# zli96/DF-GNN

Hardware: AMD Instinct MI355X
Metric: edges/s (fwd+bwd) fused GT conv, PATTERN bs=1024 dim=128 (higher is better)
Workload: dtype f32; 1 GPU; GT conv 'hyper' fwd+bwd, PATTERN-like batch bs=1024 dim=128 heads=1 (BASELINE.json configs[2]); training_pair=attn_edge in rank order (dfgnn_gt_hyper_fwd_ranked / dfgnn_gt_bwd_ranked), nodes_per_gpu=120490, edges_per_gpu=6288908, total_edges=6288908, parallelism=graph-sharded x1 (weak scaling), no data-path collective

## Files before the change

df-gnn_amd/csrc/dfgnn_dense.hpp:

```cpp
#pragma once
#include "dfgnn_block.hpp"

namespace dfgnn {

typedef _Float16 h16;
typedef __attribute__((ext_vector_type(8))) _Float16 hx8;
typedef __attribute__((ext_vector_type(4))) _Float16 hx4;
typedef __fp16 fp16x4_raw __attribute__((__vector_size__(4 * sizeof(__fp16))));
typedef __attribute__((address_space(3))) fp16x4_raw *lds_hx4_ptr;

#if defined(DFGNN_LDS_CHECK)
__attribute__((used)) static __device__ unsigned g_lds_report[4];
__device__ __forceinline__ void lds_check(const void *p, unsigned bytes, int line) {
#if defined(__HIP_DEVICE_COMPILE__)
  if (!__builtin_amdgcn_is_shared(p)) return;
  const unsigned end = (unsigned)(size_t)p + bytes;
  const unsigned lim = __builtin_amdgcn_groupstaticsize() + ((const unsigned *)__builtin_amdgcn_implicitarg_ptr())[30];
  if (end > lim && atomicAdd(&g_lds_report[0], 1u) == 0u) {
    g_lds_report[1] = (unsigned)line;
    g_lds_report[2] = end;
    g_lds_report[3] = lim;
  }
#endif
}
#define DFGNN_LDS_AT(p, bytes) ::dfgnn::lds_check((p), (bytes), __LINE__)
void lds_report_register(const void *symbol);
namespace {
struct LdsReportReg {
  LdsReportReg() { lds_report_register(HIP_SYMBOL(g_lds_report)); }
} g_lds_report_reg;
}
#else
#define DFGNN_LDS_AT(p, bytes) ((void)0)
#endif

struct Pow2Scale {
  float s, inv;
};
__device__ __forceinline__ Pow2Scale pow2_scale(float amax) {
  const int b = min(max((__builtin_amdgcn_readfirstlane(__float_as_int(amax)) >> 23) & 0xFF, 15), 254);
  return Pow2Scale{__int_as_float((268 - b) << 23), __int_as_float((b - 14) << 23)};
}
constexpr float kUnitScale = 16384.f, kUnitScaleInv = 1.f / 16384.f;

__device__ __forceinline__ void split_hx8(const float4 &a, const float4 &b, float s, hx8 &hi, hx8 &lo) {
  const float x[8] = {a.x, a.y, a.z, a.w, b.x, b.y, b.z, b.w};
#pragma unroll
  for (int j = 0; j < 8; ++j) {
    const h16 h = (h16)(x[j] * s);
    hi[j] = h;
    lo[j] = (h16)fmaf(x[j], s, -(float)h);
  }
}
__device__ __forceinline__ float absmax8(const float4 &a, const float4 &b) {
  return fmaxf(fmaxf(fmaxf(fabsf(a.x), fabsf(a.y)), fmaxf(fabsf(a.z), fabsf(a.w))),
               fmaxf(fmaxf(fabsf(b.x), fabsf(b.y)), fmaxf(fabsf(b.z), fabsf(b.w))));
}

constexpr int kDenseThreads = 512;
constexpr int kDenseWaves = kDenseThreads / kWave;
constexpr int kDenseChunkRows = 128;
constexpr int kDenseWideRows = 160;
constexpr int kDensePre = 16;

template <int F>
struct DenseCfg {
  static constexpr int RS = F + 16;
  static constexpr int KT = F / 32;
  static constexpr int FT = F / 16;
};

template <class T>
__device__ __forceinline__ const T &ld32(const T *base, unsigned idx) {
  DFGNN_LDS_AT(reinterpret_cast<const char *>(base) + (size_t)(idx * (unsigned)sizeof(T)), (unsigned)sizeof(T));
  return *reinterpret_cast<const T *>(reinterpret_cast<const char *>(base) + (size_t)(idx * (unsigned)sizeof(T)));
}
__device__ __forceinline__ float4 ld32_f4(const float *base, unsigned idx) {
  DFGNN_LDS_AT(reinterpret_cast<const char *>(base) + (size_t)(idx * 4u), 16u);
  return *reinterpret_cast<const float4 *>(reinterpret_cast<const char *>(base) + (size_t)(idx * 4u));
}
__device__ __forceinline__ void st32_f4(float *base, unsigned idx, const float4 &v) {
  DFGNN_LDS_AT(reinterpret_cast<char *>(base) + (size_t)(idx * 4u), 16u);
  *reinterpret_cast<float4 *>(reinterpret_cast<char *>(base) + (size_t)(idx * 4u)) = v;
}
#ifndef DFGNN_NT_LOADS
#define DFGNN_NT_LOADS 1
#endif
template <class T>
__device__ __forceinline__ T ld32_once(const T *base, unsigned idx) {
  const T *p = reinterpret_cast<const T *>(reinterpret_cast<const char *>(base) + (size_t)(idx * (unsigned)sizeof(T)));
#if DFGNN_NT_LOADS
  return __builtin_nontemporal_load(p);
#else
  return *p;
#endif
}
__device__ __forceinline__ float4 ld32_f4_once(const float *base, unsigned idx) {
#if DFGNN_NT_LOADS
  typedef float f4v __attribute__((ext_vector_type(4)));
  const f4v x = __builtin_nontemporal_load(reinterpret_cast<const f4v *>(reinterpret_cast<const char *>(base) + (size_t)(idx * 4u)));
  return make_float4(x[0], x[1], x[2], x[3]);
#else
  return ld32_f4(base, idx);
#endif
}
#ifndef DFGNN_NT_STORES
#define DFGNN_NT_STORES 1
#endif
__device__ __forceinline__ void st32_f4_out(float *base, unsigned idx, const float4 &v) {
#if DFGNN_NT_STORES
  typedef float f4v __attribute__((ext_vector_type(4)));
  f4v x = {v.x, v.y, v.z, v.w};
  __builtin_nontemporal_store(x, reinterpret_cast<f4v *>(reinterpret_cast<char *>(base) + (size_t)(idx * 4u)));
#else
  st32_f4(base, idx, v);
#endif
}

__device__ __forceinline__ int opaque_tid() {
  int t = threadIdx.x;
  asm volatile("" : "+v"(t));
  return t;
}
struct LaneIds {
  int mi, mq, tq, tp;
};
__device__ __forceinline__ LaneIds lane_ids() {
  int l = threadIdx.x & (kWave - 1);
  asm volatile("" : "+v"(l));
  return LaneIds{l & 15, l >> 4, (l & 15) >> 2, l & 3};
}

template <int F, int ROWS>
struct DenseStageRegs {
  static constexpr int PER = (ROWS * (F / 8) + kDenseThreads - 1) / kDenseThreads;
  float4 a[PER], b[PER];
  int row0, row_end;
};

template <int F, int ROWS, int USED = ROWS>
__device__ __forceinline__ void dense_stage_load(DenseStageRegs<F, ROWS> &r, const float *__restrict__ src, size_t hf,
                                                 int row0, int row_end, int fr = F, bool once = false) {
  constexpr int C8 = F / 8;
  const int tid = opaque_tid();
  r.row0 = row0;
  r.row_end = row_end;
#pragma unroll
  for (int k = 0; k < DenseStageRegs<F, USED>::PER; ++k) {
    const int idx = tid + k * kDenseThreads;
    const int row = min(idx / C8, USED - 1), c8 = idx % C8;
    const unsigned off = (unsigned)min(row0 + row, row_end - 1) * (unsigned)hf + ((fr >= F || 8 * c8 < fr) ? 8u * c8 : 0u);
    r.a[k] = once ? ld32_f4_once(src, off) : ld32_f4(src, off);
    r.b[k] = once ? ld32_f4_once(src, off + 4) : ld32_f4(src, off + 4);
  }
}

template <int F, int ROWS, int USED = ROWS>
__device__ __forceinline__ float dense_stage_absmax(const DenseStageRegs<F, ROWS> &r) {
  float m = 0.f;
#pragma unroll
  for (int k = 0; k < DenseStageRegs<F, USED>::PER; ++k) m = fmaxf(m, absmax8(r.a[k], r.b[k]));
  return m;
}

__device__ __forceinline__ void wg_max_post(float *slot, float v) {
  v = wave_max(v);
  DFGNN_LDS_AT(slot + threadIdx.x / kWave, 4u);
  if ((threadIdx.x & (kWave - 1)) == 0) slot[threadIdx.x / kWave] = v;
}
__device__ __forceinline__ float wg_max_read(const float *slot) {
  DFGNN_LDS_AT(slot, 32u);
  const float4 a = *reinterpret_cast<const float4 *>(slot), b = *reinterpret_cast<const float4 *>(slot + 4);
  return fmaxf(fmaxf(fmaxf(a.x, a.y), fmaxf(a.z, a.w)), fmaxf(fmaxf(b.x, b.y), fmaxf(b.z, b.w)));
}

template <int F, int ROWS, int USED = ROWS>
__device__ __forceinline__ void dense_stage_store(DenseStageRegs<F, ROWS> &r, h16 *hi, h16 *lo, float scale, int fr = F) {
  constexpr int C8 = F / 8, RS = DenseCfg<F>::RS;
  const int tid = opaque_tid();
#pragma unroll
  for (int k = 0; k < DenseStageRegs<F, USED>::PER; ++k) {
    const int idx = tid + k * kDenseThreads;
    const int row = idx / C8, c8 = idx - row * C8;
    if (idx < USED * C8) {
      const bool valid = r.row0 + row < r.row_end && (fr >= F || 8 * c8 < fr);
      const float4 z = make_float4(0.f, 0.f, 0.f, 0.f);
      hx8 h, l;
      split_hx8(valid ? r.a[k] : z, valid ? r.b[k] : z, scale, h, l);
      DFGNN_LDS_AT(hi + row * RS + 8 * c8, 16u);
      DFGNN_LDS_AT(lo + row * RS + 8 * c8, 16u);
      *reinterpret_cast<hx8 *>(hi + row * RS + 8 * c8) = h;
      *reinterpret_cast<hx8 *>(lo + row * RS + 8 * c8) = l;
    }
  }
  asm volatile("" ::: "memory");
}

template <int F>
__device__ __forceinline__ void dense_rows_frag(hx8 (&ah)[F / 32], hx8 (&al)[F / 32], const h16 *ihi,
                                                const h16 *ilo, int u, const LaneIds &L) {
  constexpr int RS = DenseCfg<F>::RS;
  const int off = (16 * u + L.mi) * RS + 8 * L.mq;
#pragma unroll
  for (int t = 0; t < F / 32; ++t) {
    DFGNN_LDS_AT(ihi + off + 32 * t, 16u);
    DFGNN_LDS_AT(ilo + off + 32 * t, 16u);
    ah[t] = *reinterpret_cast<const hx8 *>(ihi + off + 32 * t);
    al[t] = *reinterpret_cast<const hx8 *>(ilo + off + 32 * t);
  }
}
template <int F>
__device__ __forceinline__ f32x4 dense_rows_mma_frag(const hx8 (&ah)[F / 32], const hx8 (&al)[F / 32],
                                                     const hx8 (&xh)[F / 32], const hx8 (&xl)[F / 32]) {
  f32x4 acc = {0.f, 0.f, 0.f, 0.f};
#pragma unroll
  for (int t = 0; t < F / 32; ++t) {
    acc = __builtin_amdgcn_mfma_f32_16x16x32_f16(ah[t], xh[t], acc, 0, 0, 0);
    acc = __builtin_amdgcn_mfma_f32_16x16x32_f16(ah[t], xl[t], acc, 0, 0, 0);
    acc = __builtin_amdgcn_mfma_f32_16x16x32_f16(al[t], xh[t], acc, 0, 0, 0);
  }
  return acc;
}
template <int F>
__device__ __forceinline__ f32x4 dense_rows_mma(const h16 *ihi, const h16 *ilo, int u, const hx8 (&xh)[F / 32],
                                                const hx8 (&xl)[F / 32], const LaneIds &L) {
  hx8 ah[F / 32], al[F / 32];
  dense_rows_frag<F>(ah, al, ihi, ilo, u, L);
  return dense_rows_mma_frag<F>(ah, al, xh, xl);
}

template <int F, int NTILES>
__device__ __forceinline__ void dense_rows_mma_strip(f32x4 (&out)[NTILES], const h16 *ihi, const h16 *ilo, int limit,
                                                     const hx8 (&xh)[F / 32], const hx8 (&xl)[F / 32],
                                                     const LaneIds &L) {
  hx8 ah[2][F / 32], al[2][F / 32];
  dense_rows_frag<F>(ah[0], al[0], ihi, ilo, 0, L);
#pragma unroll
  for (int u = 0; u < NTILES; ++u) {
    if (u + 1 < NTILES) dense_rows_frag<F>(ah[(u + 1) & 1], al[(u + 1) & 1], ihi, ilo, u + 1, L);
    out[u] = (16 * u < limit) ? dense_rows_mma_frag<F>(ah[u & 1], al[u & 1], xh, xl) : f32x4{0.f, 0.f, 0.f, 0.f};
  }
}

__device__ __forceinline__ hx8 dense_tr_pair(const h16 *p, int second_offset) {
  DFGNN_LDS_AT(p, 8u);
  DFGNN_LDS_AT(p + second_offset, 8u);
  const hx4 a = __builtin_bit_cast(hx4, __builtin_amdgcn_ds_read_tr16_b64_v4f16((lds_hx4_ptr)(p)));
  const hx4 b = __builtin_bit_cast(hx4, __builtin_amdgcn_ds_read_tr16_b64_v4f16((lds_hx4_ptr)(p + second_offset)));
  return __builtin_shufflevector(a, b, 0, 1, 2, 3, 4, 5, 6, 7);
}

__device__ __forceinline__ void dense_split8(const f32x4 &x0, const f32x4 &x1, float scale, hx8 &h, hx8 &l) {
#pragma unroll
  for (int t = 0; t < 8; ++t) {
    const float x = (t < 4) ? x0[t] : x1[t - 4];
    const h16 hh = (h16)(x * scale);
    h[t] = hh;
    l[t] = (h16)fmaf(x, scale, -(float)hh);
  }
}

template <int F, int GMAX = 4>
__device__ __forceinline__ void dense_kblock_mma(f32x4 (&acc)[F / 16], const h16 *ihi, const h16 *ilo, int xoff,
                                                 int second, const hx8 &yh, const hx8 &yl) {
  constexpr int FT = F / 16, G = FT < GMAX ? FT : GMAX;
#pragma unroll
  for (int f0 = 0; f0 < FT; f0 += G) {
    hx8 xh[G], xl[G];
#pragma unroll
    for (int k = 0; k < G; ++k) {
      xh[k] = dense_tr_pair(ihi + xoff + 16 * (f0 + k), second);
      xl[k] = dense_tr_pair(ilo + xoff + 16 * (f0 + k), second);
    }
#pragma unroll
    for (int k = 0; k < G; ++k) acc[f0 + k] = __builtin_amdgcn_mfma_f32_16x16x32_f16(xh[k], yh, acc[f0 + k], 0, 0, 0);
#pragma unroll
    for (int k = 0; k < G; ++k) acc[f0 + k] = __builtin_amdgcn_mfma_f32_16x16x32_f16(xl[k], yh, acc[f0 + k], 0, 0, 0);
#pragma unroll
    for (int k = 0; k < G; ++k) acc[f0 + k] = __builtin_amdgcn_mfma_f32_16x16x32_f16(xh[k], yl, acc[f0 + k], 0, 0, 0);
  }
}

template <int NFT>
__device__ __forceinline__ void dense_kblock_mma2(f32x4 (&acc0)[NFT], f32x4 (&acc1)[NFT], const h16 *ihi, const h16 *ilo,
                                                  int xoff, int second, const hx8 &yh0, const hx8 &yl0, const hx8 &yh1,
                                                  const hx8 &yl1) {
  hx8 xh[NFT], xl[NFT];
#pragma unroll
  for (int k = 0; k < NFT; ++k) {
    xh[k] = dense_tr_pair(ihi + xoff + 16 * k, second);
    xl[k] = dense_tr_pair(ilo + xoff + 16 * k, second);
  }
#pragma unroll
  for (int k = 0; k < NFT; ++k) acc0[k] = __builtin_amdgcn_mfma_f32_16x16x32_f16(xh[k], yh0, acc0[k], 0, 0, 0);
#pragma unroll
  for (int k = 0; k < NFT; ++k) acc1[k] = __builtin_amdgcn_mfma_f32_16x16x32_f16(xh[k], yh1, acc1[k], 0, 0, 0);
#pragma unroll
  for (int k = 0; k < NFT; ++k) acc0[k] = __builtin_amdgcn_mfma_f32_16x16x32_f16(xl[k], yh0, acc0[k], 0, 0, 0);
#pragma unroll
  for (int k = 0; k < NFT; ++k) acc1[k] = __builtin_amdgcn_mfma_f32_16x16x32_f16(xl[k], yh1, acc1[k], 0, 0, 0);
#pragma unroll
  for (int k = 0; k < NFT; ++k) acc0[k] = __builtin_amdgcn_mfma_f32_16x16x32_f16(xh[k], yl0, acc0[k], 0, 0, 0);
#pragma unroll
  for (int k = 0; k < NFT; ++k) acc1[k] = __builtin_amdgcn_mfma_f32_16x16x32_f16(xh[k], yl1, acc1[k], 0, 0, 0);
}

template <int F, int GMAX = 4>
__device__ __forceinline__ void dense_cols_mma(f32x4 (&acc)[F / 16], const h16 *ihi, const h16 *ilo, int jb,
                                               const f32x4 &y0, const f32x4 &y1, float yscale, const LaneIds &L) {
  constexpr int RS = DenseCfg<F>::RS;
  hx8 yh, yl;
  dense_split8(y0, y1, yscale, yh, yl);
  dense_kblock_mma<F, GMAX>(acc, ihi, ilo, (32 * jb + 4 * L.mq + L.tq) * RS + 4 * L.tp, 16 * RS, yh, yl);
}

template <int NFT, bool GUARD = false, bool NT = true>
__device__ __forceinline__ void dense_store_acc(const f32x4 (&acc)[NFT], float scale, float *__restrict__ base,
                                                unsigned off, bool accumulate, int feat0 = 0, int fr = 1 << 30) {
#pragma unroll
  for (int ft = 0; ft < NFT; ++ft) {
    if constexpr (GUARD)
      if (feat0 + 16 * ft >= fr) continue;
    float4 o = make_float4(acc[ft][0] * scale, acc[ft][1] * scale, acc[ft][2] * scale, acc[ft][3] * scale);
    if (accumulate) {
      const float4 old = ld32_f4(base, off + 16 * ft);
      o.x += old.x; o.y += old.y; o.z += old.z; o.w += old.w;
    }
    if constexpr (NT) st32_f4_out(base, off + 16 * ft, o);
    else st32_f4(base, off + 16 * ft, o);
  }
}

constexpr int kDppRowRor8 = 0x128;
template <int NFT>
__device__ __forceinline__ void dense_load_rows(float4 (&prev)[NFT], const float *__restrict__ base, unsigned hf, int row, int n,
                                                const LaneIds &L) {
  const bool low = L.mi < 8;
  const int r1 = min(low ? row : row - 8, n - 1), r2 = min(low ? row + 8 : row, n - 1);
  const unsigned o1 = (unsigned)r1 * hf + (low ? 0u : 16u) + 4u * L.mq, o2 = (unsigned)r2 * hf + (low ? 16u : 0u) + 4u * L.mq;
#pragma unroll
  for (int k = 0; k < NFT / 2; ++k) {
    prev[2 * k] = ld32_f4(base, o1 + 32 * k);
    prev[2 * k + 1] = ld32_f4(base, o2 + 32 * k);
  }
}
template <int NFT, bool NT = true, bool ACC = false>
__device__ __forceinline__ void dense_store_rows(const f32x4 (&acc)[NFT], float scale, float *__restrict__ base, unsigned hf,
                                                 int row, int n, const LaneIds &L, const float4 *prev = nullptr) {
  static_assert(NFT % 2 == 0, "tiles are stored in pairs");
  const bool low = L.mi < 8;
  const int prow = low ? row + 8 : row - 8;
  const int r1 = low ? row : prow, r2 = low ? prow : row;
  const unsigned o1 = (unsigned)r1 * hf + (low ? 0u : 16u) + 4u * L.mq, o2 = (unsigned)r2 * hf + (low ? 16u : 0u) + 4u * L.mq;
#pragma unroll
  for (int k = 0; k < NFT / 2; ++k) {
    float4 a, b;
    a.x = acc[2 * k][0] * scale; a.y = acc[2 * k][1] * scale; a.z = acc[2 * k][2] * scale; a.w = acc[2 * k][3] * scale;
    b.x = dpp_perm<kDppRowRor8>(acc[2 * k + 1][0] * scale);
    b.y = dpp_perm<kDppRowRor8>(acc[2 * k + 1][1] * scale);
    b.z = dpp_perm<kDppRowRor8>(acc[2 * k + 1][2] * scale);
    b.w = dpp_perm<kDppRowRor8>(acc[2 * k + 1][3] * scale);
    float4 v1 = low ? a : b, v2 = low ? b : a;
    if constexpr (ACC) {
      const float4 p1 = prev[2 * k], p2 = prev[2 * k + 1];
      v1.x += p1.x; v1.y += p1.y; v1.z += p1.z; v1.w += p1.w;
      v2.x += p2.x; v2.y += p2.y; v2.z += p2.z; v2.w += p2.w;
    }
    if constexpr (NT) {
      if (r1 < n) st32_f4_out(base, o1 + 32 * k, v1);
      if (r2 < n) st32_f4_out(base, o2 + 32 * k, v2);
    } else {
      if (r1 < n) st32_f4(base, o1 + 32 * k, v1);
      if (r2 < n) st32_f4(base, o2 + 32 * k, v2);
    }
  }
}

__device__ __forceinline__ float xor16_32_max(float v) {
  float a = v, b = v;
  permlane32_swap(a, b);
  a = fmaxf(a, b);
  b = a;
  permlane16_swap(a, b);
  return fmaxf(a, b);
}
__device__ __forceinline__ float xor16_32_sum(float v) {
  float a = v, b = v;
  permlane32_swap(a, b);
  a += b;
  b = a;
  permlane16_swap(a, b);
  return a + b;
}

}
```

df-gnn_amd/csrc/dfgnn_dense_bwd.hpp:

```cpp
#pragma once
#include "dfgnn_dense_fwd.hpp"

namespace dfgnn {

template <int CW, int NBLK>
struct DenseBwdGeom {
  static constexpr int RB = (CW == kDenseWideRows) ? 80 : 128;
  static constexpr int RBP = (RB + 31) & ~31;
  static constexpr int U = CW / 16;
  static constexpr int TS = CW + 8;
};

struct GatBwdArgs {
  const float *edge_max, *edge_sum;
  float slope;
  float *grad_row, *grad_col;
  DenseDrop drop;
};

template <int FR, int CW, int NBLK, bool GAT = false, bool RECOMP = false, bool WEIGHTED = false>
__device__ __forceinline__ void dense_bwd_body(float *lds, const Csr &g, int n0, int n, int e0, int ne, int head,
                                               const float *__restrict__ Q, const float *__restrict__ K,
                                               const float *__restrict__ V, const float *__restrict__ attn_edge,
                                               const float *__restrict__ dO, float *__restrict__ dQ,
                                               float *__restrict__ dK, float *__restrict__ dV,
                                               const GatBwdArgs ga = GatBwdArgs{}) {
  static_assert(!(RECOMP && (GAT || CW != kDenseChunkRows)), "P is recomputed for GT, 128-column blocks");
  constexpr int F = FR < 32 ? 32 : FR;
  constexpr int fr = FR;
  using D = DenseCfg<F>;
  using G = DenseBwdGeom<CW, NBLK>;
  constexpr int RS = D::RS, KT = D::KT, FT = D::FT, RB = G::RB, RBP = G::RBP, U = G::U, TS = G::TS;
  constexpr int TB = 2 * TS;
  constexpr int PRE = GAT ? 10 : kDensePre;
  const int wave = __builtin_amdgcn_readfirstlane(threadIdx.x / kWave);
  h16 *ihi = reinterpret_cast<h16 *>(lds), *ilo = ihi + (size_t)CW * RS;
  float *T = reinterpret_cast<float *>(ilo + (size_t)CW * RS);
  h16 *Tb = reinterpret_cast<h16 *>(T);
  const size_t hf = (size_t)g.h * fr, hoff = (size_t)head * fr;
  const float *Qb = Q + (size_t)n0 * hf + hoff, *Kb = K + (size_t)n0 * hf + hoff, *Vb = V + (size_t)n0 * hf + hoff,
              *dOb = dO + (size_t)n0 * hf + hoff;
  float *dQb = dQ + (size_t)n0 * hf + hoff, *dKb = dK + (size_t)n0 * hf + hoff, *dVb = dV + (size_t)n0 * hf + hoff;
  const float *attn_h = RECOMP ? nullptr : attn_edge + (size_t)head * g.nnz;
  constexpr int SN = NBLK * CW;
  float *smax = T + RBP * TS;
  float *arl = smax + 2 * kDenseWaves, *acl = arl + SN, *mxl = acl + SN, *ivl = mxl + SN;
  (void)arl, (void)acl, (void)mxl, (void)ivl;
  DFGNN_LDS_AT(lds, (unsigned)(reinterpret_cast<char *>(GAT ? ivl + SN : arl) - reinterpret_cast<char *>(lds)));

  DFGNN_DSTAMP(0)
  if constexpr (GAT) {
    const int tid = opaque_tid();
    if (tid < SN) {
      const size_t k = (size_t)(n0 + min(tid, n - 1)) * g.h + head;
      const float a = Q[k], c = K[k], mx = ga.edge_max[k], sm = ga.edge_sum[k];
      const bool valid = tid < n;
      arl[tid] = valid ? a : 0.f;
      acl[tid] = valid ? c : 0.f;
      mxl[tid] = valid ? mx : 0.f;
      ivl[tid] = (valid && sm != 0.f) ? 1.f / sm : 0.f;
    }
  }
  DenseStageRegs<F, CW> st;
  const float *next_src = nullptr;
  int next_row0 = 0, next_end = 0;
  auto image_prefetch = [&](const float *src, int row0, int row_end, bool once = false) {
    if (NBLK > 1) {
      next_src = src;
      next_row0 = row0;
      next_end = row_end;
    } else {
      dense_stage_load<F, CW>(st, src, hf, row0, row_end, fr, once);
    }
  };
  Pow2Scale isc{1.f, 1.f};
  auto image_post = [&]() {
    if (NBLK > 1) dense_stage_load<F, CW>(st, next_src, hf, next_row0, next_end, fr);
    wg_max_post(smax, dense_stage_absmax<F, CW>(st));
  };
  auto image_store = [&]() {
    isc = pow2_scale(wg_max_read(smax));
    dense_stage_store<F, CW>(st, ihi, ilo, isc.s, fr);
  };
  unsigned pc[PRE];
  float pa[PRE];
  auto edges_prefetch = [&](int ea, int eb) {
    const int tid = opaque_tid();
#pragma unroll
    for (int k = 0; k < PRE; ++k) {
      const unsigned e = (unsigned)min(tid + k * kDenseThreads, max(eb - ea, 1) - 1);
      const int ea0 = min(ea, g.nnz - 1);
      pc[k] = ld32_once(g.coords + ea0, e);
      if constexpr (!GAT) pa[k] = ld32_once(attn_h + ea0, e);
      else pa[k] = ga.drop.mask ? ga.drop.mask[((size_t)ea0 + e) * g.h + head] : 1.f;
    }
  };
  auto gat_p = [&](int i, int j, float rnd) {
    const float pp = fast_exp(leaky_relu(arl[i] + acl[j], ga.slope) - mxl[i]) * ivl[i];
    return (rnd > ga.drop.drop) ? pp : -pp;
  };
  constexpr bool kDirectP = !GAT && NBLK == 1 && !RECOMP;
  auto put_p = [&](int i, int j, float p) {
    const h16 hh = (h16)(p * kUnitScale);
    Tb[i * TB + j] = hh;
    Tb[i * TB + TS + j] = (h16)fmaf(p, kUnitScale, -(float)hh);
  };
  auto tile_clear = [&]() {
    const int tid = opaque_tid();
    for (int k = tid; k < RBP * TS / 4; k += kDenseThreads)
      reinterpret_cast<float4 *>(T)[k] = make_float4(0.f, 0.f, 0.f, 0.f);
    lds_barrier();
  };
  auto tile_open = [&](int ea, int eb) {
    tile_clear();
    const int tid = opaque_tid();
#pragma unroll
    for (int k = 0; k < PRE; ++k) {
      const int i = pc[k] >> 8, j = pc[k] & 0xFF;
      if (tid + k * kDenseThreads < eb - ea && j < CW) {
        if constexpr (GAT) T[i * TS + j] = gat_p(i, j, pa[k]);
        else if constexpr (kDirectP) put_p(i, j, pa[k]);
        else T[i * TS + j] = pa[k];
      }
    }
  };
  auto load_tile = [&](int i0, int j0, int ea, int eb, bool opened, bool commit) {
    const int tid = opaque_tid();
    if (!opened) tile_clear();
    constexpr int B = 8;
    for (int base = opened ? PRE * kDenseThreads : 0; base < eb - ea; base += B * kDenseThreads) {
      unsigned bc[B];
      float ba[B];
#pragma unroll
      for (int k = 0; k < B; ++k) {
        const unsigned e = (unsigned)min(base + tid + k * kDenseThreads, eb - ea - 1);
        bc[k] = ld32_once(g.coords + ea, e);
        if constexpr (!GAT) ba[k] = ld32_once(attn_h + ea, e);
        else ba[k] = ga.drop.mask ? ga.drop.mask[((size_t)ea + e) * g.h + head] : 1.f;
      }
#pragma unroll
      for (int k = 0; k < B; ++k) {
        const int i = bc[k] >> 8, jj = bc[k] & 0xFF, j = jj - j0;
        if (base + tid + k * kDenseThreads < eb - ea && j >= 0 && j < CW) {
          if constexpr (GAT) T[(i - i0) * TS + j] = gat_p(i, jj, ba[k]);
          else if constexpr (kDirectP) put_p(i - i0, j, ba[k]);
          else T[(i - i0) * TS + j] = ba[k];
        }
      }
    }
    if (commit) {
      image_post();
      lds_barrier();
      image_store();
    }
    lds_barrier();
  };
  auto strip_to_tile = [&](const f32x4 (&X)[U], float tscale) {
    const LaneIds L = lane_ids();
    h16 *trow = Tb + (wave * 16 + L.mi) * TB + 4 * L.mq;
#pragma unroll
    for (int u = 0; u < U; ++u) {
      hx4 h4, l4;
#pragma unroll
      for (int r = 0; r < 4; ++r) {
        const h16 h = (h16)(X[u][r] * tscale);
        h4[r] = h;
        l4[r] = (h16)fmaf(X[u][r], tscale, -(float)h);
      }
      *reinterpret_cast<hx4 *>(trow + 16 * u) = h4;
      *reinterpret_cast<hx4 *>(trow + TS + 16 * u) = l4;
    }
  };
  auto column_strip = [&](float *outb, int j0, int cs, int ni, bool accumulate, float oscale) {
    const LaneIds L = lane_ids();
    const int j = j0 + cs * 16 + L.mi;
    f32x4 acc[FT];
#pragma unroll
    for (int ft = 0; ft < FT; ++ft) acc[ft] = f32x4{0.f, 0.f, 0.f, 0.f};
#pragma unroll
    for (int ib = 0; ib < RBP / 32; ++ib) {
      if (32 * ib < ni) {
        const int yoff = (32 * ib + 4 * L.mq + L.tq) * TB + 16 * cs + 4 * L.tp;
        const hx8 yh = dense_tr_pair(Tb + yoff, 16 * TB);
        const hx8 yl = dense_tr_pair(Tb + yoff + TS, 16 * TB);
        dense_kblock_mma<F, (NBLK == 1 ? 8 : 4)>(acc, ihi, ilo, (32 * ib + 4 * L.mq + L.tq) * RS + 4 * L.tp, 16 * RS, yh, yl);
      }
    }
    if constexpr (FR == F) {
      if (!accumulate) {
        dense_store_rows<FT>(acc, oscale, outb, (unsigned)hf, j, n, L);
        return;
      }
    }
    if (j < n) dense_store_acc<FT, (FR < F)>(acc, oscale, outb, (unsigned)j * (unsigned)hf + 4u * L.mq, accumulate, 4 * L.mq, fr);
  };
  auto column_tile = [&](float *outb, int j0, int cs, int ft, int ni, bool accumulate, float oscale) {
    const LaneIds L = lane_ids();
    const int j = j0 + cs * 16 + L.mi;
    f32x4 acc[1] = {f32x4{0.f, 0.f, 0.f, 0.f}};
#pragma unroll
    for (int ib = 0; ib < RBP / 32; ++ib) {
      if (32 * ib < ni) {
        const int yoff = (32 * ib + 4 * L.mq + L.tq) * TB + 16 * cs + 4 * L.tp;
        const hx8 yh = dense_tr_pair(Tb + yoff, 16 * TB);
        const hx8 yl = dense_tr_pair(Tb + yoff + TS, 16 * TB);
        const int xoff = (32 * ib + 4 * L.mq + L.tq) * RS + 4 * L.tp + 16 * ft;
        const hx8 xh = dense_tr_pair(ihi + xoff, 16 * RS);
        const hx8 xl = dense_tr_pair(ilo + xoff, 16 * RS);
        acc[0] = __builtin_amdgcn_mfma_f32_16x16x32_f16(xh, yh, acc[0], 0, 0, 0);
        acc[0] = __builtin_amdgcn_mfma_f32_16x16x32_f16(xl, yh, acc[0], 0, 0, 0);
        acc[0] = __builtin_amdgcn_mfma_f32_16x16x32_f16(xh, yl, acc[0], 0, 0, 0);
      }
    }
    if (j < n)
      dense_store_acc<1, (FR < F)>(acc, oscale, outb, (unsigned)j * (unsigned)hf + 16u * ft + 4u * L.mq, accumulate, 16 * ft + 4 * L.mq, fr);
  };
  constexpr bool kBlocked = NBLK == 1 && U == kDenseWaves && FR == F && FT >= 4;
  auto column_block = [&](float *outb, int ni, float oscale) {
    constexpr int NFT = kBlocked ? FT / 2 : 2;
    const LaneIds L = lane_ids();
    const int cs0 = 2 * (wave >> 1), ft0 = NFT * (wave & 1);
    f32x4 acc0[NFT], acc1[NFT];
#pragma unroll
    for (int k = 0; k < NFT; ++k) acc0[k] = acc1[k] = f32x4{0.f, 0.f, 0.f, 0.f};
#pragma unroll
    for (int ib = 0; ib < RBP / 32; ++ib) {
      if (32 * ib < ni) {
        const int yoff = (32 * ib + 4 * L.mq + L.tq) * TB + 16 * cs0 + 4 * L.tp;
        const hx8 yh0 = dense_tr_pair(Tb + yoff, 16 * TB), yl0 = dense_tr_pair(Tb + yoff + TS, 16 * TB);
        const hx8 yh1 = dense_tr_pair(Tb + yoff + 16, 16 * TB), yl1 = dense_tr_pair(Tb + yoff + 16 + TS, 16 * TB);
        dense_kblock_mma2<NFT>(acc0, acc1, ihi, ilo, (32 * ib + 4 * L.mq + L.tq) * RS + 4 * L.tp + 16 * ft0, 16 * RS, yh0,
                               yl0, yh1, yl1);
      }
    }
    dense_store_rows<NFT>(acc0, oscale, outb + 16 * ft0, (unsigned)hf, cs0 * 16 + L.mi, n, L);
    dense_store_rows<NFT>(acc1, oscale, outb + 16 * ft0, (unsigned)hf, cs0 * 16 + 16 + L.mi, n, L);
  };
  auto column_phase = [&](float *outb, int j0, int ni, bool accumulate, float oscale) {
    const int nstrips = min(U, (n - j0 + 15) >> 4);
    if constexpr (kBlocked) {
      if (2 * (wave >> 1) < nstrips) column_block(outb, ni, oscale);
      return;
    }
    if (wave < nstrips) column_strip(outb, j0, wave, ni, accumulate, oscale);
    if (U > kDenseWaves)
      for (int unit = wave; unit < (nstrips - kDenseWaves) * FT; unit += kDenseWaves)
        column_tile(outb, j0, kDenseWaves + unit / FT, unit % FT, ni, accumulate, oscale);
  };

  int ea = e0, eb = (!RECOMP && RB < n) ? g.row_ptr[n0 + RB] : e0 + ne;
  if constexpr (RECOMP) {
    image_prefetch(Kb, 0, n);
  } else {
    edges_prefetch(ea, eb);
    image_prefetch(dOb, 0, min(n, RB), !RECOMP && !GAT);
    tile_open(ea, eb);
  }
  float gcol = 0.f;
  constexpr int NRB = (NBLK * CW + RB - 1) / RB;
  for (int rb = 0; rb < NRB && rb * RB < n; ++rb) {
    const int i0 = rb * RB;
    const int ni = min(n - i0, RB);
    const bool row_wave = wave * 16 < ni;
    const bool first = i0 == 0;

    f32x4 dS[NBLK][U], Pr[NBLK][U];
    hx8 gh[KT], gl[KT];
    float doinv = 1.f;
    if constexpr (RECOMP) {
      const LaneIds L = lane_ids();
      const int irow = i0 + wave * 16 + L.mi;
      float4 qa[KT], qb[KT];
      {
        const unsigned off = (unsigned)min(irow, n - 1) * (unsigned)hf;
#pragma unroll
        for (int t = 0; t < KT; ++t) {
          const unsigned c = (FR == F || 32 * t + 8 * L.mq < fr) ? 32u * t + 8u * L.mq : 0u;
          qa[t] = ld32_f4(Qb, off + c);
          qb[t] = ld32_f4(Qb, off + c + 4);
        }
      }
      constexpr int MW = (NBLK * U + 1) / 2;
      unsigned mwd[MW];
      float smx, sinv;
      {
        const size_t node = (size_t)(n0 + min(irow, n - 1));
        const unsigned *mp = g.mask + node * kPlanMaskWords;
#pragma unroll
        for (int w = 0; w < MW; ++w) mwd[w] = (row_wave && irow < n) ? ld32(mp, (unsigned)w) : 0u;
        smx = ga.edge_max[node * g.h + head];
        const float ssum = ga.edge_sum[node * g.h + head];
        sinv = (ssum != 0.f) ? 1.f / ssum : 0.f;
      }
      hx8 qh[KT], ql[KT];
      float qinv = 1.f, lsum = 0.f;
#pragma unroll
      for (int jc = 0; jc < NBLK; ++jc) {
        if (jc > 0) image_prefetch(Kb, jc * CW, n);
        image_post();
        lds_barrier();
        image_store();
        if (jc + 1 == NBLK) image_prefetch(dOb, i0, i0 + ni);
        if (jc == 0) {
          const bool valid = row_wave && irow < n;
          float qm = 0.f;
#pragma unroll
          for (int t = 0; t < KT; ++t) {
            if (!valid || (FR < F && 32 * t + 8 * L.mq >= fr)) qa[t] = qb[t] = make_float4(0.f, 0.f, 0.f, 0.f);
            qm = fmaxf(qm, absmax8(qa[t], qb[t]));
          }
          const Pow2Scale qs = pow2_scale(wave_max(qm));
          qinv = qs.inv;
#pragma unroll
          for (int t = 0; t < KT; ++t) split_hx8(qa[t], qb[t], qs.s, qh[t], ql[t]);
        }
        lds_barrier();
        if (row_wave) {
          const int nj = n - jc * CW;
          f32x4 S[U];
          if constexpr (NBLK == 1) {
            dense_rows_mma_strip<F, U>(S, ihi, ilo, nj, qh, ql, L);
          } else {
#pragma unroll
            for (int u = 0; u < U; ++u) S[u] = (16 * u < nj) ? dense_rows_mma<F>(ihi, ilo, u, qh, ql, L) : f32x4{0.f, 0.f, 0.f, 0.f};
          }
          const float c2 = (isc.inv * qinv) * 1.4426950408889634f, b2 = smx * 1.4426950408889634f;
#pragma unroll
          for (int u = 0; u < U; ++u) {
            const int ug = jc * U + u;
            const unsigned bits = (mwd[ug / 2] >> (16 * (ug & 1) + 4 * L.mq)) & 0xFu;
            if constexpr (WEIGHTED) {
              const float4 wv = ld32_f4(g.wdense + (size_t)(n0 + min(irow, n - 1)) * kPlanWeightStride + 4 * L.mq, 16u * ug);
              S[u][0] *= wv.x; S[u][1] *= wv.y; S[u][2] *= wv.z; S[u][3] *= wv.w;
            }
#pragma unroll
            for (int r = 0; r < 4; ++r) {
              Pr[jc][u][r] = ((bits >> r) & 1u) ? __builtin_amdgcn_exp2f(fmaf(S[u][r], c2, -b2)) : 0.f;
              lsum += Pr[jc][u][r];
            }
          }
        } else {
#pragma unroll
          for (int u = 0; u < U; ++u) Pr[jc][u] = f32x4{0.f, 0.f, 0.f, 0.f};
        }
      }
      lsum = xor16_32_sum(lsum);
      const float linv = (sinv != 0.f && lsum > 0.f) ? 1.f / lsum : 0.f;
#pragma unroll
      for (int jc = 0; jc < NBLK; ++jc)
#pragma unroll
        for (int u = 0; u < U; ++u) Pr[jc][u] *= linv;
    }
#pragma unroll
    for (int jc = 0; jc < NBLK; ++jc) {
      const int j0 = jc * CW;
      if constexpr (RECOMP) {
        strip_to_tile(Pr[jc], kUnitScale);
        if (jc == 0) {
          image_post();
          lds_barrier();
          image_store();
          doinv = isc.inv;
        }
        if (jc + 1 == NBLK) image_prefetch(Vb, 0, n);
        lds_barrier();
        if (jc == 0) {
          const LaneIds L = lane_ids();
          const int off = (wave * 16 + L.mi) * RS + 8 * L.mq;
#pragma unroll
          for (int t = 0; t < KT; ++t) {
            gh[t] = row_wave ? *reinterpret_cast<const hx8 *>(ihi + off + 32 * t) : hx8{};
            gl[t] = row_wave ? *reinterpret_cast<const hx8 *>(ilo + off + 32 * t) : hx8{};
          }
        }
      } else {
      load_tile(i0, j0, ea, eb, first && jc == 0, jc == 0);
      if (jc == 0) doinv = isc.inv;
      DFGNN_DSTAMP(9)
      if (jc + 1 == NBLK) image_prefetch(Vb, 0, n);
      if (row_wave) {
        const LaneIds L = lane_ids();
        if (jc == 0) {
          const int off = (wave * 16 + L.mi) * RS + 8 * L.mq;
#pragma unroll
          for (int t = 0; t < KT; ++t) {
            gh[t] = *reinterpret_cast<const hx8 *>(ihi + off + 32 * t);
            gl[t] = *reinterpret_cast<const hx8 *>(ilo + off + 32 * t);
          }
        }
        const int nj = n - j0;
#pragma unroll
        for (int u = 0; u < U; ++u) {
          if (16 * u < nj) {
            if constexpr (kDirectP) {
              const h16 *trow = Tb + (wave * 16 + L.mi) * TB + 16 * u + 4 * L.mq;
              const hx4 h4 = *reinterpret_cast<const hx4 *>(trow), l4 = *reinterpret_cast<const hx4 *>(trow + TS);
#pragma unroll
              for (int r = 0; r < 4; ++r) Pr[jc][u][r] = ((float)h4[r] + (float)l4[r]) * kUnitScaleInv;
            } else {
              const float4 p = *reinterpret_cast<const float4 *>(T + (wave * 16 + L.mi) * TS + 16 * u + 4 * L.mq);
              Pr[jc][u] = f32x4{p.x, p.y, p.z, p.w};
            }
          } else {
            Pr[jc][u] = f32x4{0.f, 0.f, 0.f, 0.f};
          }
        }
        if constexpr (GAT) {
          f32x4 Pd[U];
#pragma unroll
          for (int u = 0; u < U; ++u)
#pragma unroll
            for (int r = 0; r < 4; ++r) Pd[u][r] = Pr[jc][u][r] > 0.f ? Pr[jc][u][r] : 0.f;
          strip_to_tile(Pd, kUnitScale);
        } else if constexpr (!kDirectP) {
          strip_to_tile(Pr[jc], kUnitScale);
        }
      } else {
#pragma unroll
        for (int u = 0; u < U; ++u) Pr[jc][u] = f32x4{0.f, 0.f, 0.f, 0.f};
        if (jc == 0) {
#pragma unroll
          for (int t = 0; t < KT; ++t) gh[t] = gl[t] = hx8{};
        }
      }
      }
      if constexpr (!kDirectP && !RECOMP) lds_barrier();
      DFGNN_DSTAMP(3)
      column_phase(dVb, j0, ni, !first, doinv * kUnitScaleInv * (GAT ? ga.drop.scale : 1.f));
      if (jc + 1 == NBLK) image_post();
      lds_barrier();
    }
    DFGNN_DSTAMP(4)

    float dpinv[NBLK];
#pragma unroll
    for (int jc = 0; jc < NBLK; ++jc) {
      image_store();
      dpinv[jc] = isc.inv * doinv;
      if (jc + 1 < NBLK) {
        image_prefetch(Vb, (jc + 1) * CW, n);
      } else if constexpr (!GAT) {
        image_prefetch(Kb, 0, n);
      } else if constexpr (CW * NBLK > RB) {
        const bool more = rb + 1 < NRB && i0 + RB < n;
        image_prefetch(dOb, more ? i0 + RB : i0, more ? min(n, i0 + 2 * RB) : i0 + 1);
      }
      lds_barrier();
      if (row_wave) {
        const LaneIds L = lane_ids();
        const int nj = n - jc * CW;
        if constexpr (NBLK == 1) {
          dense_rows_mma_strip<F, U>(dS[jc], ihi, ilo, nj, gh, gl, L);
        } else {
#pragma unroll
          for (int u = 0; u < U; ++u)
            dS[jc][u] = (16 * u < nj) ? dense_rows_mma<F>(ihi, ilo, u, gh, gl, L) : f32x4{0.f, 0.f, 0.f, 0.f};
        }
      } else {
#pragma unroll
        for (int u = 0; u < U; ++u) dS[jc][u] = f32x4{0.f, 0.f, 0.f, 0.f};
      }
      if (jc + 1 < NBLK) {
        image_post();
        lds_barrier();
      }
    }
    DFGNN_DSTAMP(1)
    float tmax = 0.f;
    if (row_wave) {
      if constexpr (GAT) {
#pragma unroll
        for (int jc = 0; jc < NBLK; ++jc)
#pragma unroll
          for (int u = 0; u < U; ++u)
#pragma unroll
            for (int r = 0; r < 4; ++r) {
              dS[jc][u][r] = Pr[jc][u][r] > 0.f ? dS[jc][u][r] * (dpinv[jc] * ga.drop.scale) : 0.f;
              Pr[jc][u][r] = fabsf(Pr[jc][u][r]);
            }
      } else {
#pragma unroll
        for (int jc = 0; jc < NBLK; ++jc)
#pragma unroll
          for (int u = 0; u < U; ++u) dS[jc][u] *= dpinv[jc];
      }
      float t = 0.f;
#pragma unroll
      for (int jc = 0; jc < NBLK; ++jc)
#pragma unroll
        for (int u = 0; u < U; ++u)
#pragma unroll
          for (int r = 0; r < 4; ++r) t = fmaf(Pr[jc][u][r], dS[jc][u][r], t);
      t = xor16_32_sum(t);
#pragma unroll
      for (int jc = 0; jc < NBLK; ++jc)
#pragma unroll
        for (int u = 0; u < U; ++u)
#pragma unroll
          for (int r = 0; r < 4; ++r) dS[jc][u][r] = Pr[jc][u][r] * (dS[jc][u][r] - t);
      if constexpr (WEIGHTED) {
        const LaneIds L = lane_ids();
        const float *wrow = g.wdense + (size_t)(n0 + min(i0 + wave * 16 + L.mi, n - 1)) * kPlanWeightStride + 4 * L.mq;
#pragma unroll
        for (int jc = 0; jc < NBLK; ++jc)
#pragma unroll
          for (int u = 0; u < U; ++u) {
            const float4 wv = ld32_f4(wrow, 16u * (jc * U + u));
            const float wvr[4] = {wv.x, wv.y, wv.z, wv.w};
#pragma unroll
            for (int r = 0; r < 4; ++r) dS[jc][u][r] = (Pr[jc][u][r] != 0.f) ? dS[jc][u][r] * wvr[r] : 0.f;
          }
      }
#pragma unroll
      for (int jc = 0; jc < NBLK; ++jc)
#pragma unroll
        for (int u = 0; u < U; ++u)
#pragma unroll
          for (int r = 0; r < 4; ++r) tmax = fmaxf(tmax, fabsf(dS[jc][u][r]));
    }
    if constexpr (!GAT) {
      wg_max_post(smax + kDenseWaves, tmax);
      image_post();
    }
    lds_barrier();
    DFGNN_DSTAMP(2)

    if constexpr (GAT) {
      float *cpart = T;
      if (rb + 1 < NRB && i0 + RB < n) {
        ea = eb;
        eb = (i0 + 2 * RB < n) ? g.row_ptr[n0 + i0 + 2 * RB] : e0 + ne;
      }
      if (row_wave) {
        const LaneIds L = lane_ids();
        const int i = i0 + wave * 16 + L.mi;
        const float ari = arl[min(i, n - 1)];
        float rs = 0.f;
#pragma unroll
        for (int jc = 0; jc < NBLK; ++jc)
#pragma unroll
          for (int u = 0; u < U; ++u) {
            const float4 a = *reinterpret_cast<const float4 *>(acl + jc * CW + 16 * u + 4 * L.mq);
            const float av[4] = {a.x, a.y, a.z, a.w};
            float cs[4];
#pragma unroll
            for (int r = 0; r < 4; ++r) {
              const float ge = dS[jc][u][r] * ((ari + av[r] > 0.f) ? 1.f : ga.slope);
              rs += ge;
              cs[r] = lanes_sum<16>(ge);
            }
            if (L.mi == 0)
              *reinterpret_cast<float4 *>(cpart + wave * SN + jc * CW + 16 * u + 4 * L.mq) = make_float4(cs[0], cs[1], cs[2], cs[3]);
          }
        rs = xor16_32_sum(rs);
        if (L.mq == 0 && i < i0 + ni) ga.grad_row[(size_t)(n0 + i) * g.h + head] = rs;
      }
      lds_barrier();
      {
        const int tid = opaque_tid();
        if (tid < SN)
          for (int w = 0; w * 16 < ni; ++w) gcol += cpart[w * SN + tid];
      }
      lds_barrier();
      continue;
    }

    f32x4 qacc[FT];
#pragma unroll
    for (int ft = 0; ft < FT; ++ft) qacc[ft] = f32x4{0.f, 0.f, 0.f, 0.f};
    const Pow2Scale ts = pow2_scale(wg_max_read(smax + kDenseWaves));
    float kinv = 1.f;
#pragma unroll
    for (int jc = 0; jc < NBLK; ++jc) {
      const int j0 = jc * CW, nj = min(n - j0, CW);
      if (row_wave) strip_to_tile(dS[jc], ts.s);
      image_store();
      if (jc > 0) {
        const float ratio = kinv * isc.s;
#pragma unroll
        for (int ft = 0; ft < FT; ++ft) qacc[ft] *= ratio;
      }
      kinv = isc.inv;
      image_prefetch(Qb, i0, i0 + ni);
      lds_barrier();
      DFGNN_DSTAMP(5)
      if constexpr (kBlocked) {
        constexpr int NFT = FT / 2;
        const int cs0 = 2 * (wave >> 1), ft0 = NFT * (wave & 1);
        if (cs0 * 16 < ni) {
          const LaneIds L = lane_ids();
          f32x4 q0[NFT], q1[NFT];
#pragma unroll
          for (int k = 0; k < NFT; ++k) q0[k] = q1[k] = f32x4{0.f, 0.f, 0.f, 0.f};
          const h16 *srow = Tb + (cs0 * 16 + L.mi) * TB + 8 * L.mq;
#pragma unroll
          for (int jb = 0; jb < CW / 32; ++jb) {
            if (32 * jb < nj) {
              const hx8 sh0 = *reinterpret_cast<const hx8 *>(srow + 32 * jb), sl0 = *reinterpret_cast<const hx8 *>(srow + TS + 32 * jb);
              const hx8 sh1 = *reinterpret_cast<const hx8 *>(srow + 16 * TB + 32 * jb),
                        sl1 = *reinterpret_cast<const hx8 *>(srow + 16 * TB + TS + 32 * jb);
              dense_kblock_mma2<NFT>(q0, q1, ihi, ilo, (32 * jb + 8 * L.mq + L.tq) * RS + 4 * L.tp + 16 * ft0, 4 * RS, sh0, sl0,
                                     sh1, sl1);
            }
          }
          dense_store_rows<NFT>(q0, kinv * ts.inv, dQb + 16 * ft0, (unsigned)hf, i0 + cs0 * 16 + L.mi, i0 + ni, L);
          dense_store_rows<NFT>(q1, kinv * ts.inv, dQb + 16 * ft0, (unsigned)hf, i0 + cs0 * 16 + 16 + L.mi, i0 + ni, L);
        }
      } else if (row_wave) {
        const LaneIds L = lane_ids();
        const h16 *srow = Tb + (wave * 16 + L.mi) * TB + 8 * L.mq;
#pragma unroll
        for (int jb = 0; jb < CW / 32; ++jb) {
          if (32 * jb < nj) {
            const hx8 sh = *reinterpret_cast<const hx8 *>(srow + 32 * jb);
            const hx8 sl = *reinterpret_cast<const hx8 *>(srow + TS + 32 * jb);
            dense_kblock_mma<F, (NBLK == 1 ? 8 : 4)>(qacc, ihi, ilo, (32 * jb + 8 * L.mq + L.tq) * RS + 4 * L.tp, 4 * RS, sh, sl);
          }
        }
        if (jc + 1 == NBLK) {
          const int i = i0 + wave * 16 + L.mi;
          if constexpr (FR == F) dense_store_rows<FT>(qacc, kinv * ts.inv, dQb, (unsigned)hf, i, i0 + ni, L);
          else if (i < i0 + ni)
            dense_store_acc<FT, true>(qacc, kinv * ts.inv, dQb, (unsigned)i * (unsigned)hf + 4u * L.mq, false, 4 * L.mq, fr);
        }
      }
      DFGNN_DSTAMP(6)
      image_post();
      lds_barrier();
      image_store();
      const float dkscale = isc.inv * ts.inv;
      if (jc + 1 < NBLK) {
        image_prefetch(Kb, (jc + 1) * CW, n);
      } else if (rb + 1 < NRB && i0 + RB < n) {
        if constexpr (RECOMP) {
          image_prefetch(Kb, 0, n);
        } else {
          ea = eb;
          eb = (i0 + 2 * RB < n) ? g.row_ptr[n0 + i0 + 2 * RB] : e0 + ne;
          image_prefetch(dOb, i0 + RB, min(n, i0 + 2 * RB));
        }
      }
      lds_barrier();
      DFGNN_DSTAMP(7)
      column_phase(dKb, j0, ni, !first, dkscale);
      if (jc + 1 < NBLK) image_post();
      lds_barrier();
    }
    DFGNN_DSTAMP(8)
  }
  if constexpr (GAT) {
    const int tid = opaque_tid();
    if (tid < n) ga.grad_col[(size_t)(n0 + tid) * g.h + head] = gcol;
  }
}

}
```

df-gnn_amd/csrc/dfgnn_dense_wide.hpp:

```cpp
#pragma once
#include <type_traits>

#include "dfgnn_dense.hpp"
#include "dfgnn_dense_stamp.hpp"
#ifndef DFGNN_RING160
#define DFGNN_RING160 2
#endif

namespace dfgnn {

#ifdef DFGNN_STAMPS
extern __device__ unsigned long long *dfgnn_dense_stamps;
#define DFGNN_WSTAMP(k)                                                                             \
  if (threadIdx.x == 0 && dfgnn_dense_stamps)                                                       \
    dfgnn_dense_stamps[((size_t)blockIdx.x * gridDim.y + blockIdx.y) * 16 + (k)] = __builtin_amdgcn_s_memtime();
#else
#define DFGNN_WSTAMP(k)
#endif

template <int FR, int NP, int R, int FWMAX = 64, bool RECOMP = false, bool WEIGHTED = false>
__device__ __forceinline__ void dense_bwd_wide_body(float *lds, const Csr &g, int n0, int n, int e0, int ne, int head,
                                                    const float *__restrict__ Q, const float *__restrict__ K,
                                                    const float *__restrict__ V, const float *__restrict__ attn_edge,
                                                    const float *__restrict__ dO, float *__restrict__ dQ,
                                                    float *__restrict__ dK, float *__restrict__ dV,
                                                    const float *__restrict__ stat_max = nullptr,
                                                    const float *__restrict__ stat_sum = nullptr) {
  constexpr int F = FR < 32 ? 32 : FR;
  constexpr int FW = F < FWMAX ? F : FWMAX;
  constexpr int NH = F / FW;
  using D = DenseCfg<FW>;
  constexpr int RS = D::RS, KT = D::KT, FT = D::FT;
  constexpr int U = NP / 16, TS = NP + 8, TB = 2 * TS, NS = (U + kDenseWaves - 1) / kDenseWaves, PRE = kDensePre;
  constexpr int QB = RECOMP ? NH : 0;
  constexpr int NQ = 4 * NH + QB;
  const int wave = __builtin_amdgcn_readfirstlane(threadIdx.x / kWave);
  const int nstrip = (n + 15) >> 4;
  h16 *ihi = reinterpret_cast<h16 *>(lds), *ilo = ihi + (size_t)NP * RS;
  float *T = reinterpret_cast<float *>(ilo + (size_t)NP * RS);
  h16 *Tb = reinterpret_cast<h16 *>(T);
  float *smax = T + NP * TS;
  DFGNN_LDS_AT(lds, (unsigned)(reinterpret_cast<char *>(smax + 2 * kDenseWaves) - reinterpret_cast<char *>(lds)));
  const size_t hf = (size_t)g.h * FR, hoff = (size_t)head * FR;
  const float *Qb = Q + (size_t)n0 * hf + hoff, *Kb = K + (size_t)n0 * hf + hoff, *Vb = V + (size_t)n0 * hf + hoff,
              *dOb = dO + (size_t)n0 * hf + hoff;
  float *dQb = dQ + (size_t)n0 * hf + hoff, *dKb = dK + (size_t)n0 * hf + hoff, *dVb = dV + (size_t)n0 * hf + hoff;
  const float *attn_h = RECOMP ? nullptr : attn_edge + (size_t)head * g.nnz + e0;
  constexpr int fr = FR < FW ? FR : FW;

  DFGNN_WSTAMP(0)
  unsigned pc[PRE];
  float pa[PRE];
  if constexpr (!RECOMP) {
    const int tid = opaque_tid();
#pragma unroll
    for (int k = 0; k < PRE; ++k) {
      const unsigned e = (unsigned)min(tid + k * kDenseThreads, max(ne, 1) - 1);
      pc[k] = ld32_once(g.coords + e0, e);
      pa[k] = ld32_once(attn_h, e);
    }
  }
  DenseStageRegs<FW, NP> st[R];
  Pow2Scale isc{1.f, 1.f};
  auto image_src = [&](int qq) -> const float * {
    if (qq < QB) return Kb + qq * FW;
    const int q = qq - QB;
    const int h = (q % (2 * NH)) / 2;
    const float *base = q < 2 * NH ? ((q & 1) ? Vb : dOb) : ((q & 1) ? Qb : Kb);
    return base + h * FW;
  };
  auto image_fetch = [&](int q) {
    const bool once = !RECOMP && q >= QB && q - QB < 2 * NH && ((q - QB) & 1) == 0;
    if (q < NQ) dense_stage_load<FW, NP>(st[q % R], image_src(q), hf, 0, n, fr, once);
  };
  auto image_post = [&](int q) { wg_max_post(smax, dense_stage_absmax<FW, NP>(st[q % R])); };
  auto image_store = [&](int q) {
    isc = pow2_scale(wg_max_read(smax));
    dense_stage_store<FW, NP>(st[q % R], ihi, ilo, isc.s, fr);
    if (q == 1) { DFGNN_WSTAMP(13) }
    image_fetch(q + R);
  };
#pragma unroll
  for (int q = 0; q < R; ++q) image_fetch(q);
  if constexpr (RECOMP) {
    float4 qa[NS][KT], qb[NS][KT];
    auto q_fetch = [&](int h) {
      const LaneIds L = lane_ids();
#pragma unroll
      for (int s = 0; s < NS; ++s) {
        const unsigned off = (unsigned)min((wave + kDenseWaves * s) * 16 + L.mi, n - 1) * (unsigned)hf + (unsigned)(h * FW);
#pragma unroll
        for (int t = 0; t < KT; ++t) {
          const unsigned c = (fr >= FW || 32 * t + 8 * L.mq < fr) ? 32u * t + 8u * L.mq : 0u;
          qa[s][t] = ld32_f4(Qb, off + c);
          qb[s][t] = ld32_f4(Qb, off + c + 4);
        }
      }
    };
    hx8 qh[NS][KT], ql[NS][KT];
    float qinv[NS];
    auto q_convert = [&]() {
      const LaneIds L = lane_ids();
#pragma unroll
      for (int s = 0; s < NS; ++s) {
        const bool valid = (wave + kDenseWaves * s) * 16 + L.mi < n;
        float qm = 0.f;
#pragma unroll
        for (int t = 0; t < KT; ++t) {
          if (!valid || (fr < FW && 32 * t + 8 * L.mq >= fr)) qa[s][t] = qb[s][t] = make_float4(0.f, 0.f, 0.f, 0.f);
          qm = fmaxf(qm, absmax8(qa[s][t], qb[s][t]));
        }
        const Pow2Scale qs = pow2_scale(wave_max(qm));
        qinv[s] = qs.inv;
#pragma unroll
        for (int t = 0; t < KT; ++t) split_hx8(qa[s][t], qb[s][t], qs.s, qh[s][t], ql[s][t]);
      }
    };
    q_fetch(0);
    constexpr int MW = (U + 1) / 2;
    unsigned mwd[NS][MW];
    float smx[NS], sinv[NS];
    {
      const LaneIds L = lane_ids();
#pragma unroll
      for (int s = 0; s < NS; ++s) {
        const int i = (wave + kDenseWaves * s) * 16 + L.mi;
        const size_t node = (size_t)(n0 + min(i, n - 1));
        const unsigned *mp = g.mask + node * kPlanMaskWords;
#pragma unroll
        for (int w = 0; w < MW; ++w) mwd[s][w] = (i < n) ? ld32(mp, (unsigned)w) : 0u;
        smx[s] = stat_max[node * g.h + head];
        const float ssum = stat_sum[node * g.h + head];
        sinv[s] = (ssum != 0.f) ? 1.f / ssum : 0.f;
      }
    }
    f32x4 S[NS][U];
#pragma unroll
    for (int s = 0; s < NS; ++s)
#pragma unroll
      for (int u = 0; u < U; ++u) S[s][u] = f32x4{0.f, 0.f, 0.f, 0.f};
#pragma unroll
    for (int h = 0; h < NH; ++h) {
      image_post(h);
      lds_barrier();
      image_store(h);
      q_convert();
      if (h + 1 < NH) q_fetch(h + 1);
      lds_barrier();
      const LaneIds L = lane_ids();
#pragma unroll
      for (int s = 0; s < NS; ++s) {
        if (wave + kDenseWaves * s < nstrip) {
          const float c = isc.inv * qinv[s];
#pragma unroll
          for (int u = 0; u < U; ++u)
            if (16 * u < n) S[s][u] += dense_rows_mma<FW>(ihi, ilo, u, qh[s], ql[s], L) * c;
        }
      }
    }
#pragma unroll
    for (int s = 0; s < NS; ++s) {
      const int strip = wave + kDenseWaves * s;
      if (strip < U) {
        const LaneIds L = lane_ids();
        h16 *trow = Tb + (strip * 16 + L.mi) * TB + 4 * L.mq;
        const float b = smx[s];
        float lsum = 0.f;
        const float *wrow = WEIGHTED ? g.wdense + (size_t)(n0 + min(strip * 16 + L.mi, n - 1)) * kPlanWeightStride + 4 * L.mq : nullptr;
#pragma unroll
        for (int u = 0; u < U; ++u) {
          const unsigned bits = (mwd[s][u / 2] >> (16 * (u & 1) + 4 * L.mq)) & 0xFu;
          if constexpr (WEIGHTED) {
            const float4 wv = ld32_f4(wrow, 16u * u);
            S[s][u][0] *= wv.x; S[s][u][1] *= wv.y; S[s][u][2] *= wv.z; S[s][u][3] *= wv.w;
          }
#pragma unroll
          for (int r = 0; r < 4; ++r) {
            S[s][u][r] = ((bits >> r) & 1u) ? fast_exp(S[s][u][r] - b) : 0.f;
            lsum += S[s][u][r];
          }
        }
        lsum = xor16_32_sum(lsum);
        const float linv = (sinv[s] != 0.f && lsum > 0.f) ? 1.f / lsum : 0.f;
#pragma unroll
        for (int u = 0; u < U; ++u) {
          hx4 h4, l4;
#pragma unroll
          for (int r = 0; r < 4; ++r) {
            const float p = S[s][u][r] * linv;
            const h16 hh = (h16)(p * kUnitScale);
            h4[r] = hh;
            l4[r] = (h16)fmaf(p, kUnitScale, -(float)hh);
          }
          *reinterpret_cast<hx4 *>(trow + 16 * u) = h4;
          *reinterpret_cast<hx4 *>(trow + TS + 16 * u) = l4;
        }
      }
    }
  } else {
    const int tid = opaque_tid();
    for (int k = tid; k < NP * TS / 4; k += kDenseThreads) reinterpret_cast<float4 *>(T)[k] = make_float4(0.f, 0.f, 0.f, 0.f);
    lds_barrier();
    auto put = [&](unsigned c, float p) {
      const int at = (int)(c >> 8) * TB + (int)(c & 0xFF);
      const h16 hh = (h16)(p * kUnitScale);
      Tb[at] = hh;
      Tb[at + TS] = (h16)fmaf(p, kUnitScale, -(float)hh);
    };
#pragma unroll
    for (int k = 0; k < PRE; ++k)
      if (tid + k * kDenseThreads < ne) put(pc[k], pa[k]);
    constexpr int B = 8;
    for (int base = PRE * kDenseThreads; base < ne; base += B * kDenseThreads) {
      unsigned bc[B];
      float ba[B];
#pragma unroll
      for (int k = 0; k < B; ++k) {
        const unsigned e = (unsigned)min(base + tid + k * kDenseThreads, ne - 1);
        bc[k] = ld32_once(g.coords + e0, e);
        ba[k] = ld32_once(attn_h, e);
      }
#pragma unroll
      for (int k = 0; k < B; ++k)
        if (base + tid + k * kDenseThreads < ne) put(bc[k], ba[k]);
    }
  }
  image_post(QB);
  lds_barrier();
  image_store(QB);
  lds_barrier();
  DFGNN_WSTAMP(1)

  auto column_unit = [&](float *outb, int cs, int ft, float oscale) {
    const LaneIds L = lane_ids();
    const int j = cs * 16 + L.mi;
    if (ft < 0) {
      f32x4 acc[FT];
#pragma unroll
      for (int t = 0; t < FT; ++t) acc[t] = f32x4{0.f, 0.f, 0.f, 0.f};
#pragma unroll
      for (int ib = 0; ib < NP / 32; ++ib) {
        if (32 * ib < n) {
          const int yoff = (32 * ib + 4 * L.mq + L.tq) * TB + 16 * cs + 4 * L.tp;
          const hx8 yh = dense_tr_pair(Tb + yoff, 16 * TB);
          const hx8 yl = dense_tr_pair(Tb + yoff + TS, 16 * TB);
          dense_kblock_mma<FW, (FW > 64 ? 8 : 4)>(acc, ihi, ilo, (32 * ib + 4 * L.mq + L.tq) * RS + 4 * L.tp, 16 * RS, yh, yl);
        }
      }
      if constexpr (FR == F) dense_store_rows<FT>(acc, oscale, outb, (unsigned)hf, j, n, L);
      else if (j < n) dense_store_acc<FT, true>(acc, oscale, outb, (unsigned)j * (unsigned)hf + 4u * L.mq, false, 4 * L.mq, fr);
    } else {
      f32x4 acc[1] = {f32x4{0.f, 0.f, 0.f, 0.f}};
#pragma unroll
      for (int ib = 0; ib < NP / 32; ++ib) {
        if (32 * ib < n) {
          const int yoff = (32 * ib + 4 * L.mq + L.tq) * TB + 16 * cs + 4 * L.tp;
          const hx8 yh = dense_tr_pair(Tb + yoff, 16 * TB);
          const hx8 yl = dense_tr_pair(Tb + yoff + TS, 16 * TB);
          const int xoff = (32 * ib + 4 * L.mq + L.tq) * RS + 4 * L.tp + 16 * ft;
          const hx8 xh = dense_tr_pair(ihi + xoff, 16 * RS);
          const hx8 xl = dense_tr_pair(ilo + xoff, 16 * RS);
          acc[0] = __builtin_amdgcn_mfma_f32_16x16x32_f16(xh, yh, acc[0], 0, 0, 0);
          acc[0] = __builtin_amdgcn_mfma_f32_16x16x32_f16(xl, yh, acc[0], 0, 0, 0);
          acc[0] = __builtin_amdgcn_mfma_f32_16x16x32_f16(xh, yl, acc[0], 0, 0, 0);
        }
      }
      if (j < n)
        dense_store_acc<1, (FR < F)>(acc, oscale, outb, (unsigned)j * (unsigned)hf + 16u * ft + 4u * L.mq, false, 16 * ft + 4 * L.mq, fr);
    }
  };
  auto column_phase = [&](float *outb, float oscale) {
    if (wave < nstrip) column_unit(outb, wave, -1, oscale);
    for (int unit = wave; unit < (nstrip - kDenseWaves) * FT; unit += kDenseWaves)
      column_unit(outb, kDenseWaves + unit / FT, unit % FT, oscale);
  };

  f32x4 dP[NS][U];
#pragma unroll
  for (int s = 0; s < NS; ++s)
#pragma unroll
    for (int u = 0; u < U; ++u) dP[s][u] = f32x4{0.f, 0.f, 0.f, 0.f};
#pragma unroll
  for (int h = 0; h < NH; ++h) {
    const float doinv = isc.inv;
    hx8 gh[NS][KT], gl[NS][KT];
#pragma unroll
    for (int s = 0; s < NS; ++s) {
      const LaneIds L = lane_ids();
      const int strip = wave + kDenseWaves * s;
      const int off = (min(strip, U - 1) * 16 + L.mi) * RS + 8 * L.mq;
#pragma unroll
      for (int t = 0; t < KT; ++t) {
        gh[s][t] = *reinterpret_cast<const hx8 *>(ihi + off + 32 * t);
        gl[s][t] = *reinterpret_cast<const hx8 *>(ilo + off + 32 * t);
      }
    }
    column_phase(dVb + h * FW, doinv * kUnitScaleInv);
    if (h == 0) { DFGNN_WSTAMP(2) }
    image_post(QB + 2 * h + 1);
    lds_barrier();
    if (h == 0) { DFGNN_WSTAMP(12) }
    image_store(QB + 2 * h + 1);
    if (h == 0) { DFGNN_WSTAMP(14) }
    lds_barrier();
    if (h == 0) { DFGNN_WSTAMP(3) }
    {
      const float c = isc.inv * doinv;
      const LaneIds L = lane_ids();
#pragma unroll
      for (int s = 0; s < NS; ++s) {
        if (wave + kDenseWaves * s < nstrip) {
#pragma unroll
          for (int u = 0; u < U; ++u) {
            if (16 * u < n) {
              const f32x4 a = dense_rows_mma<FW>(ihi, ilo, u, gh[s], gl[s], L);
              dP[s][u] += a * c;
            }
          }
        }
      }
    }
    if (h == 0) { DFGNN_WSTAMP(4) }
    if (h + 1 < NH) {
      image_post(QB + 2 * h + 2);
      lds_barrier();
      image_store(QB + 2 * h + 2);
      lds_barrier();
    }
  }

  DFGNN_WSTAMP(5)
  float tmax = 0.f;
#pragma unroll
  for (int s = 0; s < NS; ++s) {
    const int strip = wave + kDenseWaves * s;
    if (strip < nstrip) {
      const LaneIds L = lane_ids();
      const h16 *prow = Tb + (strip * 16 + L.mi) * TB + 4 * L.mq;
      float t = 0.f;
#pragma unroll
      for (int u = 0; u < U; ++u) {
        const hx4 ph = *reinterpret_cast<const hx4 *>(prow + 16 * u), pl = *reinterpret_cast<const hx4 *>(prow + TS + 16 * u);
#pragma unroll
        for (int r = 0; r < 4; ++r) t = fmaf(((float)ph[r] + (float)pl[r]) * kUnitScaleInv, dP[s][u][r], t);
      }
      t = xor16_32_sum(t);
#pragma unroll
      for (int u = 0; u < U; ++u) {
        const hx4 ph = *reinterpret_cast<const hx4 *>(prow + 16 * u), pl = *reinterpret_cast<const hx4 *>(prow + TS + 16 * u);
        float4 wv = make_float4(1.f, 1.f, 1.f, 1.f);
        if constexpr (WEIGHTED)
          wv = ld32_f4(g.wdense + (size_t)(n0 + min(strip * 16 + L.mi, n - 1)) * kPlanWeightStride + 4 * L.mq, 16u * u);
        const float wvr[4] = {wv.x, wv.y, wv.z, wv.w};
#pragma unroll
        for (int r = 0; r < 4; ++r) {
          const float p = ((float)ph[r] + (float)pl[r]) * kUnitScaleInv;
          dP[s][u][r] = p * (dP[s][u][r] - t);
          if constexpr (WEIGHTED) dP[s][u][r] = (p != 0.f) ? dP[s][u][r] * wvr[r] : 0.f;
          tmax = fmaxf(tmax, fabsf(dP[s][u][r]));
        }
      }
    }
  }
  DFGNN_WSTAMP(6)
  wg_max_post(smax + kDenseWaves, tmax);
  image_post(QB + 2 * NH);
  lds_barrier();
  const Pow2Scale ts = pow2_scale(wg_max_read(smax + kDenseWaves));
#pragma unroll
  for (int s = 0; s < NS; ++s) {
    const int strip = wave + kDenseWaves * s;
    if (strip < nstrip) {
      const LaneIds L = lane_ids();
      h16 *trow = Tb + (strip * 16 + L.mi) * TB + 4 * L.mq;
#pragma unroll
      for (int u = 0; u < U; ++u) {
        hx4 h4, l4;
#pragma unroll
        for (int r = 0; r < 4; ++r) {
          const h16 hh = (h16)(dP[s][u][r] * ts.s);
          h4[r] = hh;
          l4[r] = (h16)fmaf(dP[s][u][r], ts.s, -(float)hh);
        }
        *reinterpret_cast<hx4 *>(trow + 16 * u) = h4;
        *reinterpret_cast<hx4 *>(trow + TS + 16 * u) = l4;
      }
    }
  }
  image_store(QB + 2 * NH);
  lds_barrier();
  DFGNN_WSTAMP(7)

#pragma unroll
  for (int h = 0; h < NH; ++h) {
#pragma unroll
    for (int s = 0; s < NS; ++s) {
      const int strip = wave + kDenseWaves * s;
      if (strip < nstrip) {
        const LaneIds L = lane_ids();
        f32x4 qacc[FT];
#pragma unroll
        for (int t = 0; t < FT; ++t) qacc[t] = f32x4{0.f, 0.f, 0.f, 0.f};
        const h16 *srow = Tb + (strip * 16 + L.mi) * TB + 8 * L.mq;
#pragma unroll
        for (int jb = 0; jb < NP / 32; ++jb) {
          if (32 * jb < n) {
            const hx8 sh = *reinterpret_cast<const hx8 *>(srow + 32 * jb);
            const hx8 sl = *reinterpret_cast<const hx8 *>(srow + TS + 32 * jb);
            dense_kblock_mma<FW, (FW > 64 ? 8 : 4)>(qacc, ihi, ilo, (32 * jb + 8 * L.mq + L.tq) * RS + 4 * L.tp, 4 * RS, sh, sl);
          }
        }
        const int i = strip * 16 + L.mi;
        if constexpr (FR == F) dense_store_rows<FT>(qacc, isc.inv * ts.inv, dQb + h * FW, (unsigned)hf, i, n, L);
        else if (i < n)
          dense_store_acc<FT, true>(qacc, isc.inv * ts.inv, dQb + h * FW, (unsigned)i * (unsigned)hf + 4u * L.mq, false, 4 * L.mq, fr);
      }
    }
    if (h == 0) { DFGNN_WSTAMP(8) }
    image_post(QB + 2 * NH + 2 * h + 1);
    lds_barrier();
    image_store(QB + 2 * NH + 2 * h + 1);
    lds_barrier();
    if (h == 0) { DFGNN_WSTAMP(9) }
    column_phase(dKb + h * FW, isc.inv * ts.inv);
    if (h == 0) { DFGNN_WSTAMP(10) }
    if (h + 1 < NH) {
      image_post(QB + 2 * NH + 2 * h + 2);
      lds_barrier();
      image_store(QB + 2 * NH + 2 * h + 2);
      lds_barrier();
    }
  }
  DFGNN_WSTAMP(11)
}

constexpr int kDenseWide2Rows = 192;
#ifndef DFGNN_RING192
#define DFGNN_RING192 2
#endif

template <int FR, int R = DFGNN_RING192>
__device__ __forceinline__ void dense_bwd_wide2_body(float *lds, const Csr &g, int n0, int n, int e0, int ne,
                                                     const float *__restrict__ Q, const float *__restrict__ K,
                                                     const float *__restrict__ V, const float *__restrict__ attn_edge,
                                                     const float *__restrict__ dO, float *__restrict__ dQ,
                                                     float *__restrict__ dK, float *__restrict__ dV) {
  static_assert(FR == 64 || FR == 128, "one head of 64 or 128 features");
  constexpr int FW = 64, NH = FR / FW;
  using D = DenseCfg<FW>;
  constexpr int RS = D::RS, KT = D::KT, FT = D::FT;
  constexpr int NC = kDenseWide2Rows, RB = NC / 2, U = NC / 16, TS = NC + 8, TB = 2 * TS, PRE = kDensePre;
  constexpr int NQ = 4 * NH;
  const int wave = __builtin_amdgcn_readfirstlane(threadIdx.x / kWave);
  const int ncs = (n + 15) >> 4;
  h16 *ihi = reinterpret_cast<h16 *>(lds), *ilo = ihi + (size_t)NC * RS;
  float *T = reinterpret_cast<float *>(ilo + (size_t)NC * RS);
  h16 *Tb = reinterpret_cast<h16 *>(T);
  float *smax = T + RB * TS;
  DFGNN_LDS_AT(lds, (unsigned)(reinterpret_cast<char *>(smax + 2 * kDenseWaves) - reinterpret_cast<char *>(lds)));
  constexpr unsigned hf = FR;
  const float *Qb = Q + (size_t)n0 * hf, *Kb = K + (size_t)n0 * hf, *Vb = V + (size_t)n0 * hf, *dOb = dO + (size_t)n0 * hf;
  float *dQb = dQ + (size_t)n0 * hf, *dKb = dK + (size_t)n0 * hf, *dVb = dV + (size_t)n0 * hf;
  const int e1 = g.row_ptr[n0 + min(n, RB)];

  unsigned pc[PRE];
  float pa[PRE];
  auto edges_prefetch = [&](int ea, int cnt) {
    const int tid = opaque_tid();
    const int ea0 = min(ea, g.nnz - 1);
#pragma unroll
    for (int k = 0; k < PRE; ++k) {
      const unsigned e = (unsigned)min(tid + k * kDenseThreads, max(cnt, 1) - 1);
      pc[k] = ld32_once(g.coords + ea0, e);
      pa[k] = ld32_once(attn_edge + ea0, e);
    }
  };
  auto scatter = [&](int i0, int ea, int cnt) {
    const int tid = opaque_tid();
    auto put = [&](unsigned c, float p) {
      const int at = ((int)(c >> 8) - i0) * TB + (int)(c & 0xFF);
      const h16 hh = (h16)(p * kUnitScale);
      Tb[at] = hh;
      Tb[at + TS] = (h16)fmaf(p, kUnitScale, -(float)hh);
    };
#pragma unroll
    for (int k = 0; k < PRE; ++k)
      if (tid + k * kDenseThreads < cnt) put(pc[k], pa[k]);
    constexpr int B = 8;
    for (int base = PRE * kDenseThreads; base < cnt; base += B * kDenseThreads) {
      unsigned bc[B];
      float ba[B];
#pragma unroll
      for (int k = 0; k < B; ++k) {
        const unsigned e = (unsigned)min(base + tid + k * kDenseThreads, cnt - 1);
        bc[k] = ld32_once(g.coords + ea, e);
        ba[k] = ld32_once(attn_edge + ea, e);
      }
#pragma unroll
      for (int k = 0; k < B; ++k)
        if (base + tid + k * kDenseThreads < cnt) put(bc[k], ba[k]);
    }
  };

  DenseStageRegs<FW, NC> st[R];
  Pow2Scale isc{1.f, 1.f};
  auto image_rows = [](int gq) { const int q = gq % NQ; return (q < 2 * NH) == ((q & 1) == 0); };
  auto image_fetch = [&](int gq) {
    if (gq >= 2 * NQ) return;
    const int q = gq % NQ, h = (q % (2 * NH)) / 2;
    const int i0 = (gq / NQ) * RB, i1 = min(n, i0 + RB);
    if (q < 2 * NH) {
      if (q & 1) dense_stage_load<FW, NC>(st[gq % R], Vb + h * FW, hf, 0, n);
      else dense_stage_load<FW, NC, RB>(st[gq % R], dOb + h * FW, hf, i0, i1, FW, true);
    } else {
      if (q & 1) dense_stage_load<FW, NC, RB>(st[gq % R], Qb + h * FW, hf, i0, i1);
      else dense_stage_load<FW, NC>(st[gq % R], Kb + h * FW, hf, 0, n);
    }
  };
  auto image_post = [&](int gq) {
    wg_max_post(smax, image_rows(gq) ? dense_stage_absmax<FW, NC, RB>(st[gq % R]) : dense_stage_absmax<FW, NC>(st[gq % R]));
  };
  auto image_store = [&](int gq) {
    isc = pow2_scale(wg_max_read(smax));
    if (image_rows(gq)) dense_stage_store<FW, NC, RB>(st[gq % R], ihi, ilo, isc.s);
    else dense_stage_store<FW, NC>(st[gq % R], ihi, ilo, isc.s);
    image_fetch(gq + R);
  };

  float4 pvs[FT], pvt[2];
  auto prev_fetch = [&](const float *outb) {
    const LaneIds L = lane_ids();
    dense_load_rows<FT>(pvs, outb, hf, min(wave, ncs - 1) * 16 + L.mi, n, L);
#pragma unroll
    for (int k = 0; k < 2; ++k) {
      const int unit = min(wave + k * kDenseWaves, max(ncs - kDenseWaves, 1) * FT - 1);
      const int j = min((kDenseWaves + unit / FT) * 16 + L.mi, n - 1);
      pvt[k] = ld32_f4(outb, (unsigned)j * hf + 16u * (unit % FT) + 4u * L.mq);
    }
  };
  auto column_unit = [&](float *outb, int cs, int ft, int k, int ni, float oscale, auto accc) {
    constexpr bool ACC = decltype(accc)::value;
    const LaneIds L = lane_ids();
    const int j = cs * 16 + L.mi;
    if (ft < 0) {
      f32x4 acc[FT];
#pragma unroll
      for (int t = 0; t < FT; ++t) acc[t] = f32x4{0.f, 0.f, 0.f, 0.f};
#pragma unroll
      for (int ib = 0; ib < RB / 32; ++ib) {
        if (32 * ib < ni) {
          const int yoff = (32 * ib + 4 * L.mq + L.tq) * TB + 16 * cs + 4 * L.tp;
          const hx8 yh = dense_tr_pair(Tb + yoff, 16 * TB);
          const hx8 yl = dense_tr_pair(Tb + yoff + TS, 16 * TB);
          dense_kblock_mma<FW, 4>(acc, ihi, ilo, (32 * ib + 4 * L.mq + L.tq) * RS + 4 * L.tp, 16 * RS, yh, yl);
        }
      }
      dense_store_rows<FT, ACC, ACC>(acc, oscale, outb, hf, j, n, L, pvs);
    } else {
      f32x4 acc[1] = {f32x4{0.f, 0.f, 0.f, 0.f}};
#pragma unroll
      for (int ib = 0; ib < RB / 32; ++ib) {
        if (32 * ib < ni) {
          const int yoff = (32 * ib + 4 * L.mq + L.tq) * TB + 16 * cs + 4 * L.tp;
          const hx8 yh = dense_tr_pair(Tb + yoff, 16 * TB);
          const hx8 yl = dense_tr_pair(Tb + yoff + TS, 16 * TB);
          const int xoff = (32 * ib + 4 * L.mq + L.tq) * RS + 4 * L.tp + 16 * ft;
          const hx8 xh = dense_tr_pair(ihi + xoff, 16 * RS);
          const hx8 xl = dense_tr_pair(ilo + xoff, 16 * RS);
          acc[0] = __builtin_amdgcn_mfma_f32_16x16x32_f16(xh, yh, acc[0], 0, 0, 0);
          acc[0] = __builtin_amdgcn_mfma_f32_16x16x32_f16(xl, yh, acc[0], 0, 0, 0);
          acc[0] = __builtin_amdgcn_mfma_f32_16x16x32_f16(xh, yl, acc[0], 0, 0, 0);
        }
      }
      if (j < n) {
        const unsigned off = (unsigned)j * hf + 16u * ft + 4u * L.mq;
        if constexpr (ACC) {
          const float4 old = pvt[k];
          st32_f4_out(outb, off, make_float4(fmaf(acc[0][0], oscale, old.x), fmaf(acc[0][1], oscale, old.y),
                                             fmaf(acc[0][2], oscale, old.z), fmaf(acc[0][3], oscale, old.w)));
        } else {
          dense_store_acc<1, false, false>(acc, oscale, outb, off, false);
        }
      }
    }
  };
  auto column_phase = [&](float *outb, int ni, float oscale, auto accc) {
    if (wave < ncs) column_unit(outb, wave, -1, 0, ni, oscale, accc);
#pragma unroll
    for (int k = 0; k < 2; ++k) {
      const int unit = wave + k * kDenseWaves;
      if (unit < (ncs - kDenseWaves) * FT) column_unit(outb, kDenseWaves + unit / FT, unit % FT, k, ni, oscale, accc);
    }
  };

  edges_prefetch(e0, e1 - e0);
#pragma unroll
  for (int q = 0; q < R; ++q) image_fetch(q);

  auto row_block = [&](auto rbc) {
    constexpr int rb = decltype(rbc)::value, q0 = rb * NQ;
    constexpr std::integral_constant<bool, (rb > 0)> onto{};
    const int i0 = rb * RB, ni = min(n - i0, RB);
    const bool row_wave = wave * 16 < ni;
    if (rb > 0) lds_barrier();
    {
      const int tid = opaque_tid();
      for (int k = tid; k < RB * TS / 4; k += kDenseThreads) reinterpret_cast<float4 *>(T)[k] = make_float4(0.f, 0.f, 0.f, 0.f);
    }
    lds_barrier();
    if (rb == 0) scatter(0, e0, e1 - e0);
    else scatter(i0, e1, e0 + ne - e1);
    image_post(q0);
    lds_barrier();
    if constexpr (rb > 0) prev_fetch(dVb);
    image_store(q0);
    lds_barrier();

    f32x4 dP[U];
#pragma unroll
    for (int u = 0; u < U; ++u) dP[u] = f32x4{0.f, 0.f, 0.f, 0.f};
#pragma unroll
    for (int h = 0; h < NH; ++h) {
      const float doinv = isc.inv;
      hx8 gh[KT], gl[KT];
      {
        const LaneIds L = lane_ids();
        const int off = (min(wave, RB / 16 - 1) * 16 + L.mi) * RS + 8 * L.mq;
#pragma unroll
        for (int t = 0; t < KT; ++t) {
          gh[t] = *reinterpret_cast<const hx8 *>(ihi + off + 32 * t);
          gl[t] = *reinterpret_cast<const hx8 *>(ilo + off + 32 * t);
        }
      }
      column_phase(dVb + h * FW, ni, doinv * kUnitScaleInv, onto);
      image_post(q0 + 2 * h + 1);
      lds_barrier();
      image_store(q0 + 2 * h + 1);
      lds_barrier();
      if (row_wave) {
        const float c = isc.inv * doinv;
        const LaneIds L = lane_ids();
#pragma unroll
        for (int u = 0; u < U; ++u)
          if (16 * u < n) dP[u] += dense_rows_mma<FW>(ihi, ilo, u, gh, gl, L) * c;
      }
      if (h + 1 < NH) {
        image_post(q0 + 2 * h + 2);
        lds_barrier();
        if constexpr (rb > 0) prev_fetch(dVb + (h + 1) * FW);
        image_store(q0 + 2 * h + 2);
        lds_barrier();
      }
    }

    float tmax = 0.f;
    if (row_wave) {
      const LaneIds L = lane_ids();
      const h16 *prow = Tb + (wave * 16 + L.mi) * TB + 4 * L.mq;
      float t = 0.f;
#pragma unroll
      for (int u = 0; u < U; ++u) {
        const hx4 ph = *reinterpret_cast<const hx4 *>(prow + 16 * u), pl = *reinterpret_cast<const hx4 *>(prow + TS + 16 * u);
#pragma unroll
        for (int r = 0; r < 4; ++r) t = fmaf(((float)ph[r] + (float)pl[r]) * kUnitScaleInv, dP[u][r], t);
      }
      t = xor16_32_sum(t);
#pragma unroll
      for (int u = 0; u < U; ++u) {
        const hx4 ph = *reinterpret_cast<const hx4 *>(prow + 16 * u), pl = *reinterpret_cast<const hx4 *>(prow + TS + 16 * u);
#pragma unroll
        for (int r = 0; r < 4; ++r) {
          dP[u][r] = ((float)ph[r] + (float)pl[r]) * kUnitScaleInv * (dP[u][r] - t);
          tmax = fmaxf(tmax, fabsf(dP[u][r]));
        }
      }
    }
    wg_max_post(smax + kDenseWaves, tmax);
    image_post(q0 + 2 * NH);
    lds_barrier();
    const Pow2Scale ts = pow2_scale(wg_max_read(smax + kDenseWaves));
    if (row_wave) {
      const LaneIds L = lane_ids();
      h16 *trow = Tb + (wave * 16 + L.mi) * TB + 4 * L.mq;
#pragma unroll
      for (int u = 0; u < U; ++u) {
        hx4 h4, l4;
#pragma unroll
        for (int r = 0; r < 4; ++r) {
          const h16 hh = (h16)(dP[u][r] * ts.s);
          h4[r] = hh;
          l4[r] = (h16)fmaf(dP[u][r], ts.s, -(float)hh);
        }
        *reinterpret_cast<hx4 *>(trow + 16 * u) = h4;
        *reinterpret_cast<hx4 *>(trow + TS + 16 * u) = l4;
      }
    }
    image_store(q0 + 2 * NH);
    lds_barrier();

#pragma unroll
    for (int h = 0; h < NH; ++h) {
      if (row_wave) {
        const LaneIds L = lane_ids();
        f32x4 qacc[FT];
#pragma unroll
        for (int t = 0; t < FT; ++t) qacc[t] = f32x4{0.f, 0.f, 0.f, 0.f};
        const h16 *srow = Tb + (wave * 16 + L.mi) * TB + 8 * L.mq;
#pragma unroll
        for (int jb = 0; jb < NC / 32; ++jb) {
          if (32 * jb < n) {
            const hx8 sh = *reinterpret_cast<const hx8 *>(srow + 32 * jb);
            const hx8 sl = *reinterpret_cast<const hx8 *>(srow + TS + 32 * jb);
            dense_kblock_mma<FW, 4>(qacc, ihi, ilo, (32 * jb + 8 * L.mq + L.tq) * RS + 4 * L.tp, 4 * RS, sh, sl);
          }
        }
        dense_store_rows<FT>(qacc, isc.inv * ts.inv, dQb + h * FW, hf, i0 + wave * 16 + L.mi, i0 + ni, L);
      }
      image_post(q0 + 2 * NH + 2 * h + 1);
      lds_barrier();
      if constexpr (rb > 0) prev_fetch(dKb + h * FW);
      image_store(q0 + 2 * NH + 2 * h + 1);
      lds_barrier();
      if (rb == 0 && h + 1 == NH) edges_prefetch(e1, e0 + ne - e1);
      column_phase(dKb + h * FW, ni, isc.inv * ts.inv, onto);
      if (h + 1 < NH) {
        image_post(q0 + 2 * NH + 2 * h + 2);
        lds_barrier();
        image_store(q0 + 2 * NH + 2 * h + 2);
        lds_barrier();
      }
    }
  };
  row_block(std::integral_constant<int, 0>{});
  row_block(std::integral_constant<int, 1>{});
}

}
```

Measured before the change: 31.24 billion edges/s.

## Swizzle LDS tile and K-image row layouts to reduce bank conflicts

Adds a shared LDS layout header that XOR-swizzles column offsets in the P/dS tile and optionally permutes row order in the staged K image. All tile writes, transposed reads and row reads in the backward and wide kernels now go through these helpers, and the row reads are split into two 4-wide loads. The aim is to cut LDS bank conflicts in the ds_read_tr and MFMA operand loads. The cost is extra index arithmetic, plus narrower loads that may raise the LDS instruction count.

```diff
diff --git a/df-gnn_amd/csrc/dfgnn_dense.hpp b/df-gnn_amd/csrc/dfgnn_dense.hpp
--- a/df-gnn_amd/csrc/dfgnn_dense.hpp
+++ b/df-gnn_amd/csrc/dfgnn_dense.hpp
@@ -1,5 +1,6 @@
 #pragma once
 #include "dfgnn_block.hpp"
+#include "dfgnn_lds_layout.hpp"
 
 namespace dfgnn {
 
@@ -175,8 +176,10 @@
 }
 
 template <int F, int ROWS, int USED = ROWS>
-__device__ __forceinline__ void dense_stage_store(DenseStageRegs<F, ROWS> &r, h16 *hi, h16 *lo, float scale, int fr = F) {
+__device__ __forceinline__ void dense_stage_store(DenseStageRegs<F, ROWS> &r, h16 *hi, h16 *lo, float scale, int fr = F,
+                                                  bool kswap = false) {
   constexpr int C8 = F / 8, RS = DenseCfg<F>::RS;
+  static_assert(RS == image_rs(F), "the image layout of dfgnn_lds_layout.hpp");
   const int tid = opaque_tid();
 #pragma unroll
   for (int k = 0; k < DenseStageRegs<F, USED>::PER; ++k) {
@@ -187,10 +190,11 @@
       const float4 z = make_float4(0.f, 0.f, 0.f, 0.f);
       hx8 h, l;
       split_hx8(valid ? r.a[k] : z, valid ? r.b[k] : z, scale, h, l);
-      DFGNN_LDS_AT(hi + row * RS + 8 * c8, 16u);
-      DFGNN_LDS_AT(lo + row * RS + 8 * c8, 16u);
-      *reinterpret_cast<hx8 *>(hi + row * RS + 8 * c8) = h;
-      *reinterpret_cast<hx8 *>(lo + row * RS + 8 * c8) = l;
+      const int irow = image_row(row, kswap);
+      DFGNN_LDS_AT(hi + irow * RS + 8 * c8, 16u);
+      DFGNN_LDS_AT(lo + irow * RS + 8 * c8, 16u);
+      *reinterpret_cast<hx8 *>(hi + irow * RS + 8 * c8) = h;
+      *reinterpret_cast<hx8 *>(lo + irow * RS + 8 * c8) = l;
     }
   }
   asm volatile("" ::: "memory");
@@ -248,6 +252,41 @@
   const hx4 a = __builtin_bit_cast(hx4, __builtin_amdgcn_ds_read_tr16_b64_v4f16((lds_hx4_ptr)(p)));
   const hx4 b = __builtin_bit_cast(hx4, __builtin_amdgcn_ds_read_tr16_b64_v4f16((lds_hx4_ptr)(p + second_offset)));
   return __builtin_shufflevector(a, b, 0, 1, 2, 3, 4, 5, 6, 7);
+}
+
+template <int TS>
+__device__ __forceinline__ int tile_strip_off(int strip, const LaneIds &L) {
+  return tile_at(TS, L.mi, 4 * L.mq, 0) + strip * 16 * 2 * TS;
+}
+template <int TS>
+__device__ __forceinline__ int tile_tr_off(int cs, const LaneIds &L) {
+  return tile_at(TS, 4 * L.mq + L.tq, 4 * L.tp, 0) + 16 * cs;
+}
+template <int TS>
+__device__ __forceinline__ int tile_row_off(int strip, int part, const LaneIds &L) {
+  return tile_at(TS, L.mi, 8 * L.mq + 4 * part, 0) + strip * 16 * 2 * TS;
+}
+__device__ __forceinline__ hx8 tile_row8(const h16 *a, const h16 *b) {
+  DFGNN_LDS_AT(a, 8u);
+  DFGNN_LDS_AT(b, 8u);
+  return __builtin_shufflevector(*reinterpret_cast<const hx4 *>(a), *reinterpret_cast<const hx4 *>(b), 0, 1, 2, 3, 4, 5, 6, 7);
+}
+template <int TS>
+__device__ __forceinline__ void tile_put_p(h16 *Tb, int i, int j, float p) {
+  const int at = tile_at(TS, i, j, 0);
+  const h16 hh = (h16)(p * kUnitScale);
+  DFGNN_LDS_AT(Tb + at + TS, 2u);
+  Tb[at] = hh;
+  Tb[at + TS] = (h16)fmaf(p, kUnitScale, -(float)hh);
+}
+struct KImageOff {
+  int first, second;
+};
+template <int RS>
+__device__ __forceinline__ KImageOff image_k_off(const LaneIds &L) {
+  const int r = 8 * (L.mq & 3) + L.tq;
+  const int a = image_at(RS, 0, r, 4 * L.tp, 0, true);
+  return KImageOff{a, image_at(RS, 0, r + 4, 4 * L.tp, 0, true) - a};
 }
 
 __device__ __forceinline__ void dense_split8(const f32x4 &x0, const f32x4 &x1, float scale, hx8 &h, hx8 &l) {
diff --git a/df-gnn_amd/csrc/dfgnn_dense_bwd.hpp b/df-gnn_amd/csrc/dfgnn_dense_bwd.hpp
--- a/df-gnn_amd/csrc/dfgnn_dense_bwd.hpp
+++ b/df-gnn_amd/csrc/dfgnn_dense_bwd.hpp
@@ -8,7 +8,7 @@
   static constexpr int RB = (CW == kDenseWideRows) ? 80 : 128;
   static constexpr int RBP = (RB + 31) & ~31;
   static constexpr int U = CW / 16;
-  static constexpr int TS = CW + 8;
+  static constexpr int TS = tile_ts(CW);
 };
 
 struct GatBwdArgs {
@@ -78,9 +78,9 @@
     if (NBLK > 1) dense_stage_load<F, CW>(st, next_src, hf, next_row0, next_end, fr);
     wg_max_post(smax, dense_stage_absmax<F, CW>(st));
   };
-  auto image_store = [&]() {
+  auto image_store = [&](bool kswap = false) {
     isc = pow2_scale(wg_max_read(smax));
-    dense_stage_store<F, CW>(st, ihi, ilo, isc.s, fr);
+    dense_stage_store<F, CW>(st, ihi, ilo, isc.s, fr, kswap);
   };
   unsigned pc[PRE];
   float pa[PRE];
@@ -100,14 +100,10 @@
     return (rnd > ga.drop.drop) ? pp : -pp;
   };
   constexpr bool kDirectP = !GAT && NBLK == 1 && !RECOMP;
-  auto put_p = [&](int i, int j, float p) {
-    const h16 hh = (h16)(p * kUnitScale);
-    Tb[i * TB + j] = hh;
-    Tb[i * TB + TS + j] = (h16)fmaf(p, kUnitScale, -(float)hh);
-  };
+  auto put_p = [&](int i, int j, float p) { tile_put_p<TS>(Tb, i, j, p); };
   auto tile_clear = [&]() {
     const int tid = opaque_tid();
-    for (int k = tid; k < RBP * TS / 4; k += kDenseThreads)
+    for (int k = tid; k < tile_elems(TS, RBP) / 8; k += kDenseThreads)
       reinterpret_cast<float4 *>(T)[k] = make_float4(0.f, 0.f, 0.f, 0.f);
     lds_barrier();
   };
@@ -157,7 +153,7 @@
   };
   auto strip_to_tile = [&](const f32x4 (&X)[U], float tscale) {
     const LaneIds L = lane_ids();
-    h16 *trow = Tb + (wave * 16 + L.mi) * TB + 4 * L.mq;
+    h16 *trow = Tb + tile_strip_off<TS>(wave, L);
 #pragma unroll
     for (int u = 0; u < U; ++u) {
       hx4 h4, l4;
@@ -180,7 +176,7 @@
 #pragma unroll
     for (int ib = 0; ib < RBP / 32; ++ib) {
       if (32 * ib < ni) {
-        const int yoff = (32 * ib + 4 * L.mq + L.tq) * TB + 16 * cs + 4 * L.tp;
+        const int yoff = tile_tr_off<TS>(cs, L) + 32 * ib * TB;
         const hx8 yh = dense_tr_pair(Tb + yoff, 16 * TB);
         const hx8 yl = dense_tr_pair(Tb + yoff + TS, 16 * TB);
         dense_kblock_mma<F, (NBLK == 1 ? 8 : 4)>(acc, ihi, ilo, (32 * ib + 4 * L.mq + L.tq) * RS + 4 * L.tp, 16 * RS, yh, yl);
@@ -201,7 +197,7 @@
 #pragma unroll
     for (int ib = 0; ib < RBP / 32; ++ib) {
       if (32 * ib < ni) {
-        const int yoff = (32 * ib + 4 * L.mq + L.tq) * TB + 16 * cs + 4 * L.tp;
+        const int yoff = tile_tr_off<TS>(cs, L) + 32 * ib * TB;
         const hx8 yh = dense_tr_pair(Tb + yoff, 16 * TB);
         const hx8 yl = dense_tr_pair(Tb + yoff + TS, 16 * TB);
         const int xoff = (32 * ib + 4 * L.mq + L.tq) * RS + 4 * L.tp + 16 * ft;
@@ -226,7 +222,7 @@
 #pragma unroll
     for (int ib = 0; ib < RBP / 32; ++ib) {
       if (32 * ib < ni) {
-        const int yoff = (32 * ib + 4 * L.mq + L.tq) * TB + 16 * cs0 + 4 * L.tp;
+        const int yoff = tile_tr_off<TS>(cs0, L) + 32 * ib * TB;
         const hx8 yh0 = dense_tr_pair(Tb + yoff, 16 * TB), yl0 = dense_tr_pair(Tb + yoff + TS, 16 * TB);
         const hx8 yh1 = dense_tr_pair(Tb + yoff + 16, 16 * TB), yl1 = dense_tr_pair(Tb + yoff + 16 + TS, 16 * TB);
         dense_kblock_mma2<NFT>(acc0, acc1, ihi, ilo, (32 * ib + 4 * L.mq + L.tq) * RS + 4 * L.tp + 16 * ft0, 16 * RS, yh0,
@@ -393,7 +389,7 @@
         for (int u = 0; u < U; ++u) {
           if (16 * u < nj) {
             if constexpr (kDirectP) {
-              const h16 *trow = Tb + (wave * 16 + L.mi) * TB + 16 * u + 4 * L.mq;
+              const h16 *trow = Tb + tile_strip_off<TS>(wave, L) + 16 * u;
               const hx4 h4 = *reinterpret_cast<const hx4 *>(trow), l4 = *reinterpret_cast<const hx4 *>(trow + TS);
 #pragma unroll
               for (int r = 0; r < 4; ++r) Pr[jc][u][r] = ((float)h4[r] + (float)l4[r]) * kUnitScaleInv;
@@ -574,7 +570,7 @@
     for (int jc = 0; jc < NBLK; ++jc) {
       const int j0 = jc * CW, nj = min(n - j0, CW);
       if (row_wave) strip_to_tile(dS[jc], ts.s);
-      image_store();
+      image_store(true);
       if (jc > 0) {
         const float ratio = kinv * isc.s;
 #pragma unroll
@@ -592,15 +588,15 @@
           f32x4 q0[NFT], q1[NFT];
 #pragma unroll
           for (int k = 0; k < NFT; ++k) q0[k] = q1[k] = f32x4{0.f, 0.f, 0.f, 0.f};
-          const h16 *srow = Tb + (cs0 * 16 + L.mi) * TB + 8 * L.mq;
+          const h16 *sa = Tb + tile_row_off<TS>(cs0, 0, L), *sb = Tb + tile_row_off<TS>(cs0, 1, L);
+          const KImageOff ko = image_k_off<RS>(L);
 #pragma unroll
           for (int jb = 0; jb < CW / 32; ++jb) {
             if (32 * jb < nj) {
-              const hx8 sh0 = *reinterpret_cast<const hx8 *>(srow + 32 * jb), sl0 = *reinterpret_cast<const hx8 *>(srow + TS + 32 * jb);
-              const hx8 sh1 = *reinterpret_cast<const hx8 *>(srow + 16 * TB + 32 * jb),
-                        sl1 = *reinterpret_cast<const hx8 *>(srow + 16 * TB + TS + 32 * jb);
-              dense_kblock_mma2<NFT>(q0, q1, ihi, ilo, (32 * jb + 8 * L.mq + L.tq) * RS + 4 * L.tp + 16 * ft0, 4 * RS, sh0, sl0,
-                                     sh1, sl1);
+              const hx8 sh0 = tile_row8(sa + 32 * jb, sb + 32 * jb), sl0 = tile_row8(sa + TS + 32 * jb, sb + TS + 32 * jb);
+              const hx8 sh1 = tile_row8(sa + 16 * TB + 32 * jb, sb + 16 * TB + 32 * jb),
+                        sl1 = tile_row8(sa + 16 * TB + TS + 32 * jb, sb + 16 * TB + TS + 32 * jb);
+              dense_kblock_mma2<NFT>(q0, q1, ihi, ilo, ko.first + 32 * jb * RS + 16 * ft0, ko.second, sh0, sl0, sh1, sl1);
             }
           }
           dense_store_rows<NFT>(q0, kinv * ts.inv, dQb + 16 * ft0, (unsigned)hf, i0 + cs0 * 16 + L.mi, i0 + ni, L);
@@ -608,13 +604,14 @@
         }
       } else if (row_wave) {
         const LaneIds L = lane_ids();
-        const h16 *srow = Tb + (wave * 16 + L.mi) * TB + 8 * L.mq;
+        const h16 *sa = Tb + tile_row_off<TS>(wave, 0, L), *sb = Tb + tile_row_off<TS>(wave, 1, L);
+        const KImageOff ko = image_k_off<RS>(L);
 #pragma unroll
         for (int jb = 0; jb < CW / 32; ++jb) {
           if (32 * jb < nj) {
-            const hx8 sh = *reinterpret_cast<const hx8 *>(srow + 32 * jb);
-            const hx8 sl = *reinterpret_cast<const hx8 *>(srow + TS + 32 * jb);
-            dense_kblock_mma<F, (NBLK == 1 ? 8 : 4)>(qacc, ihi, ilo, (32 * jb + 8 * L.mq + L.tq) * RS + 4 * L.tp, 4 * RS, sh, sl);
+            const hx8 sh = tile_row8(sa + 32 * jb, sb + 32 * jb);
+            const hx8 sl = tile_row8(sa + TS + 32 * jb, sb + TS + 32 * jb);
+            dense_kblock_mma<F, (NBLK == 1 ? 8 : 4)>(qacc, ihi, ilo, ko.first + 32 * jb * RS, ko.second, sh, sl);
           }
         }
         if (jc + 1 == NBLK) {
diff --git a/df-gnn_amd/csrc/dfgnn_dense_wide.hpp b/df-gnn_amd/csrc/dfgnn_dense_wide.hpp
--- a/df-gnn_amd/csrc/dfgnn_dense_wide.hpp
+++ b/df-gnn_amd/csrc/dfgnn_dense_wide.hpp
@@ -31,7 +31,7 @@
   constexpr int NH = F / FW;
   using D = DenseCfg<FW>;
   constexpr int RS = D::RS, KT = D::KT, FT = D::FT;
-  constexpr int U = NP / 16, TS = NP + 8, TB = 2 * TS, NS = (U + kDenseWaves - 1) / kDenseWaves, PRE = kDensePre;
+  constexpr int U = NP / 16, TS = tile_ts(NP), TB = 2 * TS, NS = (U + kDenseWaves - 1) / kDenseWaves, PRE = kDensePre;
   constexpr int QB = RECOMP ? NH : 0;
   constexpr int NQ = 4 * NH + QB;
   const int wave = __builtin_amdgcn_readfirstlane(threadIdx.x / kWave);
@@ -74,9 +74,9 @@
     if (q < NQ) dense_stage_load<FW, NP>(st[q % R], image_src(q), hf, 0, n, fr, once);
   };
   auto image_post = [&](int q) { wg_max_post(smax, dense_stage_absmax<FW, NP>(st[q % R])); };
-  auto image_store = [&](int q) {
+  auto image_store = [&](int q, bool kswap = false) {
     isc = pow2_scale(wg_max_read(smax));
-    dense_stage_store<FW, NP>(st[q % R], ihi, ilo, isc.s, fr);
+    dense_stage_store<FW, NP>(st[q % R], ihi, ilo, isc.s, fr, kswap);
     if (q == 1) { DFGNN_WSTAMP(13) }
     image_fetch(q + R);
   };
@@ -163,7 +163,7 @@
       const int strip = wave + kDenseWaves * s;
       if (strip < U) {
         const LaneIds L = lane_ids();
-        h16 *trow = Tb + (strip * 16 + L.mi) * TB + 4 * L.mq;
+        h16 *trow = Tb + tile_strip_off<TS>(strip, L);
         const float b = smx[s];
         float lsum = 0.f;
         const float *wrow = WEIGHTED ? g.wdense + (size_t)(n0 + min(strip * 16 + L.mi, n - 1)) * kPlanWeightStride + 4 * L.mq : nullptr;
@@ -199,14 +199,9 @@
     }
   } else {
     const int tid = opaque_tid();
-    for (int k = tid; k < NP * TS / 4; k += kDenseThreads) reinterpret_cast<float4 *>(T)[k] = make_float4(0.f, 0.f, 0.f, 0.f);
-    lds_barrier();
-    auto put = [&](unsigned c, float p) {
-      const int at = (int)(c >> 8) * TB + (int)(c & 0xFF);
-      const h16 hh = (h16)(p * kUnitScale);
-      Tb[at] = hh;
-      Tb[at + TS] = (h16)fmaf(p, kUnitScale, -(float)hh);
-    };
+    for (int k = tid; k < tile_elems(TS, NP) / 8; k += kDenseThreads) reinterpret_cast<float4 *>(T)[k] = make_float4(0.f, 0.f, 0.f, 0.f);
+    lds_barrier();
+    auto put = [&](unsigned c, float p) { tile_put_p<TS>(Tb, (int)(c >> 8), (int)(c & 0xFF), p); };
 #pragma unroll
     for (int k = 0; k < PRE; ++k)
       if (tid + k * kDenseThreads < ne) put(pc[k], pa[k]);
@@ -241,7 +236,7 @@
 #pragma unroll
       for (int ib = 0; ib < NP / 32; ++ib) {
         if (32 * ib < n) {
-          const int yoff = (32 * ib + 4 * L.mq + L.tq) * TB + 16 * cs + 4 * L.tp;
+          const int yoff = tile_tr_off<TS>(cs, L) + 32 * ib * TB;
           const hx8 yh = dense_tr_pair(Tb + yoff, 16 * TB);
           const hx8 yl = dense_tr_pair(Tb + yoff + TS, 16 * TB);
           dense_kblock_mma<FW, (FW > 64 ? 8 : 4)>(acc, ihi, ilo, (32 * ib + 4 * L.mq + L.tq) * RS + 4 * L.tp, 16 * RS, yh, yl);
@@ -254,7 +249,7 @@
 #pragma unroll
       for (int ib = 0; ib < NP / 32; ++ib) {
         if (32 * ib < n) {
-          const int yoff = (32 * ib + 4 * L.mq + L.tq) * TB + 16 * cs + 4 * L.tp;
+          const int yoff = tile_tr_off<TS>(cs, L) + 32 * ib * TB;
           const hx8 yh = dense_tr_pair(Tb + yoff, 16 * TB);
           const hx8 yl = dense_tr_pair(Tb + yoff + TS, 16 * TB);
           const int xoff = (32 * ib + 4 * L.mq + L.tq) * RS + 4 * L.tp + 16 * ft;
@@ -336,7 +331,7 @@
     const int strip = wave + kDenseWaves * s;
     if (strip < nstrip) {
       const LaneIds L = lane_ids();
-      const h16 *prow = Tb + (strip * 16 + L.mi) * TB + 4 * L.mq;
+      const h16 *prow = Tb + tile_strip_off<TS>(strip, L);
       float t = 0.f;
 #pragma unroll
       for (int u = 0; u < U; ++u) {
@@ -372,7 +367,7 @@
     const int strip = wave + kDenseWaves * s;
     if (strip < nstrip) {
       const LaneIds L = lane_ids();
-      h16 *trow = Tb + (strip * 16 + L.mi) * TB + 4 * L.mq;
+      h16 *trow = Tb + tile_strip_off<TS>(strip, L);
 #pragma unroll
       for (int u = 0; u < U; ++u) {
         hx4 h4, l4;
@@ -387,7 +382,7 @@
       }
     }
   }
-  image_store(QB + 2 * NH);
+  image_store(QB + 2 * NH, true);
   lds_barrier();
   DFGNN_WSTAMP(7)
 
@@ -401,13 +396,14 @@
         f32x4 qacc[FT];
 #pragma unroll
         for (int t = 0; t < FT; ++t) qacc[t] = f32x4{0.f, 0.f, 0.f, 0.f};
-        const h16 *srow = Tb + (strip * 16 + L.mi) * TB + 8 * L.mq;
+        const h16 *sa = Tb + tile_row_off<TS>(strip, 0, L), *sb = Tb + tile_row_off<TS>(strip, 1, L);
+        const KImageOff ko = image_k_off<RS>(L);
 #pragma unroll
         for (int jb = 0; jb < NP / 32; ++jb) {
           if (32 * jb < n) {
-            const hx8 sh = *reinterpret_cast<const hx8 *>(srow + 32 * jb);
-            const hx8 sl = *reinterpret_cast<const hx8 *>(srow + TS + 32 * jb);
-            dense_kblock_mma<FW, (FW > 64 ? 8 : 4)>(qacc, ihi, ilo, (32 * jb + 8 * L.mq + L.tq) * RS + 4 * L.tp, 4 * RS, sh, sl);
+            const hx8 sh = tile_row8(sa + 32 * jb, sb + 32 * jb);
+            const hx8 sl = tile_row8(sa + TS + 32 * jb, sb + TS + 32 * jb);
+            dense_kblock_mma<FW, (FW > 64 ? 8 : 4)>(qacc, ihi, ilo, ko.first + 32 * jb * RS, ko.second, sh, sl);
           }
         }
         const int i = strip * 16 + L.mi;
@@ -427,7 +423,7 @@
     if (h + 1 < NH) {
       image_post(QB + 2 * NH + 2 * h + 2);
       lds_barrier();
-      image_store(QB + 2 * NH + 2 * h + 2);
+      image_store(QB + 2 * NH + 2 * h + 2, true);
       lds_barrier();
     }
   }
@@ -449,7 +445,7 @@
   constexpr int FW = 64, NH = FR / FW;
   using D = DenseCfg<FW>;
   constexpr int RS = D::RS, KT = D::KT, FT = D::FT;
-  constexpr int NC = kDenseWide2Rows, RB = NC / 2, U = NC / 16, TS = NC + 8, TB = 2 * TS, PRE = kDensePre;
+  constexpr int NC = kDenseWide2Rows, RB = NC / 2, U = NC / 16, TS = tile_ts(NC), TB = 2 * TS, PRE = kDensePre;
   constexpr int NQ = 4 * NH;
   const int wave = __builtin_amdgcn_readfirstlane(threadIdx.x / kWave);
   const int ncs = (n + 15) >> 4;
@@ -477,12 +473,7 @@
   };
   auto scatter = [&](int i0, int ea, int cnt) {
     const int tid = opaque_tid();
-    auto put = [&](unsigned c, float p) {
-      const int at = ((int)(c >> 8) - i0) * TB + (int)(c & 0xFF);
-      const h16 hh = (h16)(p * kUnitScale);
-      Tb[at] = hh;
-      Tb[at + TS] = (h16)fmaf(p, kUnitScale, -(float)hh);
-    };
+    auto put = [&](unsigned c, float p) { tile_put_p<TS>(Tb, (int)(c >> 8) - i0, (int)(c & 0xFF), p); };
 #pragma unroll
     for (int k = 0; k < PRE; ++k)
       if (tid + k * kDenseThreads < cnt) put(pc[k], pa[k]);
@@ -520,10 +511,10 @@
   auto image_post = [&](int gq) {
     wg_max_post(smax, image_rows(gq) ? dense_stage_absmax<FW, NC, RB>(st[gq % R]) : dense_stage_absmax<FW, NC>(st[gq % R]));
   };
-  auto image_store = [&](int gq) {
+  auto image_store = [&](int gq, bool kswap = false) {
     isc = pow2_scale(wg_max_read(smax));
     if (image_rows(gq)) dense_stage_store<FW, NC, RB>(st[gq % R], ihi, ilo, isc.s);
-    else dense_stage_store<FW, NC>(st[gq % R], ihi, ilo, isc.s);
+    else dense_stage_store<FW, NC>(st[gq % R], ihi, ilo, isc.s, FW, kswap);
     image_fetch(gq + R);
   };
 
@@ -549,7 +540,7 @@
 #pragma unroll
       for (int ib = 0; ib < RB / 32; ++ib) {
         if (32 * ib < ni) {
-          const int yoff = (32 * ib + 4 * L.mq + L.tq) * TB + 16 * cs + 4 * L.tp;
+          const int yoff = tile_tr_off<TS>(cs, L) + 32 * ib * TB;
           const hx8 yh = dense_tr_pair(Tb + yoff, 16 * TB);
           const hx8 yl = dense_tr_pair(Tb + yoff + TS, 16 * TB);
           dense_kblock_mma<FW, 4>(acc, ihi, ilo, (32 * ib + 4 * L.mq + L.tq) * RS + 4 * L.tp, 16 * RS, yh, yl);
@@ -561,7 +552,7 @@
 #pragma unroll
       for (int ib = 0; ib < RB / 32; ++ib) {
         if (32 * ib < ni) {
-          const int yoff = (32 * ib + 4 * L.mq + L.tq) * TB + 16 * cs + 4 * L.tp;
+          const int yoff = tile_tr_off<TS>(cs, L) + 32 * ib * TB;
           const hx8 yh = dense_tr_pair(Tb + yoff, 16 * TB);
           const hx8 yl = dense_tr_pair(Tb + yoff + TS, 16 * TB);
           const int xoff = (32 * ib + 4 * L.mq + L.tq) * RS + 4 * L.tp + 16 * ft;
@@ -605,7 +596,7 @@
     if (rb > 0) lds_barrier();
     {
       const int tid = opaque_tid();
-      for (int k = tid; k < RB * TS / 4; k += kDenseThreads) reinterpret_cast<float4 *>(T)[k] = make_float4(0.f, 0.f, 0.f, 0.f);
+      for (int k = tid; k < tile_elems(TS, RB) / 8; k += kDenseThreads) reinterpret_cast<float4 *>(T)[k] = make_float4(0.f, 0.f, 0.f, 0.f);
     }
     lds_barrier();
     if (rb == 0) scatter(0, e0, e1 - e0);
@@ -656,7 +647,7 @@
     float tmax = 0.f;
     if (row_wave) {
       const LaneIds L = lane_ids();
-      const h16 *prow = Tb + (wave * 16 + L.mi) * TB + 4 * L.mq;
+      const h16 *prow = Tb + tile_strip_off<TS>(wave, L);
       float t = 0.f;
 #pragma unroll
       for (int u = 0; u < U; ++u) {
@@ -681,7 +672,7 @@
     const Pow2Scale ts = pow2_scale(wg_max_read(smax + kDenseWaves));
     if (row_wave) {
       const LaneIds L = lane_ids();
-      h16 *trow = Tb + (wave * 16 + L.mi) * TB + 4 * L.mq;
+      h16 *trow = Tb + tile_strip_off<TS>(wave, L);
 #pragma unroll
       for (int u = 0; u < U; ++u) {
         hx4 h4, l4;
@@ -695,7 +686,7 @@
         *reinterpret_cast<hx4 *>(trow + TS + 16 * u) = l4;
       }
     }
-    image_store(q0 + 2 * NH);
+    image_store(q0 + 2 * NH, true);
     lds_barrier();
 
 #pragma unroll
@@ -705,13 +696,14 @@
         f32x4 qacc[FT];
 #pragma unroll
         for (int t = 0; t < FT; ++t) qacc[t] = f32x4{0.f, 0.f, 0.f, 0.f};
-        const h16 *srow = Tb + (wave * 16 + L.mi) * TB + 8 * L.mq;
+        const h16 *sa = Tb + tile_row_off<TS>(wave, 0, L), *sb = Tb + tile_row_off<TS>(wave, 1, L);
+        const KImageOff ko = image_k_off<RS>(L);
 #pragma unroll
         for (int jb = 0; jb < NC / 32; ++jb) {
           if (32 * jb < n) {
-            const hx8 sh = *reinterpret_cast<const hx8 *>(srow + 32 * jb);
-            const hx8 sl = *reinterpret_cast<const hx8 *>(srow + TS + 32 * jb);
-            dense_kblock_mma<FW, 4>(qacc, ihi, ilo, (32 * jb + 8 * L.mq + L.tq) * RS + 4 * L.tp, 4 * RS, sh, sl);
+            const hx8 sh = tile_row8(sa + 32 * jb, sb + 32 * jb);
+            const hx8 sl = tile_row8(sa + TS + 32 * jb, sb + TS + 32 * jb);
+            dense_kblock_mma<FW, 4>(qacc, ihi, ilo, ko.first + 32 * jb * RS, ko.second, sh, sl);
           }
         }
         dense_store_rows<FT>(qacc, isc.inv * ts.inv, dQb + h * FW, hf, i0 + wave * 16 + L.mi, i0 + ni, L);
@@ -726,7 +718,7 @@
       if (h + 1 < NH) {
         image_post(q0 + 2 * NH + 2 * h + 2);
         lds_barrier();
-        image_store(q0 + 2 * NH + 2 * h + 2);
+        image_store(q0 + 2 * NH + 2 * h + 2, true);
         lds_barrier();
       }
     }
diff --git a/df-gnn_amd/csrc/dfgnn_lds_layout.hpp b/df-gnn_amd/csrc/dfgnn_lds_layout.hpp
--- /dev/null
+++ b/df-gnn_amd/csrc/dfgnn_lds_layout.hpp
@@ -0,0 +1,25 @@
+#pragma once
+
+#if defined(__HIPCC__) || defined(__CUDACC__)
+#define DFGNN_LAYOUT_FN __host__ __device__ constexpr
+#else
+#define DFGNN_LAYOUT_FN constexpr
+#endif
+
+namespace dfgnn {
+
+DFGNN_LAYOUT_FN int tile_ts(int columns) { return columns + 8; }
+DFGNN_LAYOUT_FN int tile_elems(int ts, int rows) { return rows * 2 * ts; }
+DFGNN_LAYOUT_FN int tile_swizzle(int row) { return (row & 12) ^ ((row >> 1) & 4); }
+DFGNN_LAYOUT_FN int tile_at(int ts, int row, int col, int half) { return row * 2 * ts + (col ^ tile_swizzle(row)) + half * ts; }
+
+DFGNN_LAYOUT_FN int image_rs(int f) { return f + 16; }
+DFGNN_LAYOUT_FN int image_row(int row, bool kswap) { return kswap ? row ^ ((row >> 1) & 4) : row; }
+DFGNN_LAYOUT_FN int image_at(int rs, int rows, int row, int feat, int half, bool kswap = false) {
+  return half * rows * rs + image_row(row, kswap) * rs + feat;
+}
+
+static_assert(tile_at(136, 16 + 5, 32 + 12, 1) == tile_at(136, 5, 12, 1) + 16 * 272 + 32, "tile_at is periodic");
+static_assert(image_at(144, 128, 32 + 9, 20, 0, true) == image_at(144, 128, 9, 20, 0, true) + 32 * 144, "image_at is periodic");
+
+}
```

New measurement: 31.64 billion edges/s (median of 6 runs). 1.01x the previous value.
